# TXH-mercury/VALOR

Hardware: AMD Instinct MI355X
Metric: pretrain samples/sec (V+A+T clip) (higher is better)
Workload: dtype bf16

## Files before the change

### include/valor_hip.h

```cpp
#ifndef VALOR_HIP_H
#define VALOR_HIP_H
#include <stdint.h>
#ifdef __cplusplus
extern "C" {
#endif

#define VALOR_DT_BF16 0
#define VALOR_DT_F32 1
#define VALOR_OK 0
#define VALOR_ERR_ARG (-1)
#define VALOR_ERR_LAUNCH (-2)
#define VALOR_ACT_NONE 0
#define VALOR_ACT_GELU_ERF 1
#define VALOR_ACT_QUICK_GELU 2
#define VALOR_ACT_RELU 3
#define VALOR_ACT_TANH 4
#define VALOR_ACT_DERIV 16

int valor_gemm(void* stream, int dtype, int transA, int transB, int M, int N, int K, const void* A, int64_t lda,
               const void* B, int64_t ldb, void* C, int64_t ldc, const void* bias, int act, void* preact,
               const void* dact_aux, int64_t ldaux, float alpha, int accumulate, int out_f32, void* workspace,
               int64_t workspace_bytes, void* rowsum_out,
               int rowsum_accumulate);

typedef struct valor_gemm_policy {
    int key[12];
    int variant;
    int tr_asm;
    int fast_epilogue;
    int sched_256;
    int sched_narrow;
} valor_gemm_policy;
int valor_gemm_tuned(const valor_gemm_policy* policy, void* stream, int dtype, int transA, int transB, int M, int N, int K,
                     const void* A, int64_t lda, const void* B, int64_t ldb, void* C, int64_t ldc, const void* bias, int act,
                     void* preact, const void* dact_aux, int64_t ldaux, float alpha, int accumulate, int out_f32, void* workspace,
                     int64_t workspace_bytes, void* rowsum_out, int rowsum_accumulate);
int valor_gemm_kernel_for_tuned(const valor_gemm_policy* policy, int dtype, int transA, int transB, int M, int N, int K,
                                int heavy_epilogue);

typedef struct valor_gemm_pending { unsigned char opaque[256]; } valor_gemm_pending;
int valor_gemm_deferred(void* stream, int dtype, int transA, int transB, int M, int N, int K, const void* A, int64_t lda,
                        const void* B, int64_t ldb, void* C, int64_t ldc, const void* bias, int act, void* preact,
                        const void* dact_aux, int64_t ldaux, float alpha, int accumulate, int out_f32, void* workspace,
                        int64_t workspace_bytes, void* rowsum_out, int rowsum_accumulate, valor_gemm_pending* pending);
int valor_gemm_pending_bytes(const valor_gemm_pending* pending, int64_t* bytes);
int valor_gemm_reduce_group(void* stream, int dtype, const valor_gemm_pending* pendings, int n);

int valor_gemm_set_variant(int v);
int valor_gemm_kernel_for(int dtype, int transA, int transB, int M, int N, int K, int heavy_epilogue);
int valor_gemm_set_tr_asm(int v);
int valor_gemm_set_fast_epilogue(int v);
int valor_gemm_set_policy(int key, int value);
int valor_gemm_set_8ph_sched(int v);
int valor_gemm_set_narrow_sched(int v);
int valor_gemm_narrow_occupancy(void);
int valor_gemm_wide_occupancy(void);

typedef struct valor_xattn_seg {
    const void* q; const void* o; const void* dout; void* dq; const float* lse; const int* kv_range;
    int64_t q_bs, q_rs, o_bs, o_rs, do_bs, do_rs, dq_bs, dq_rs;
    int B, Sq;
    uint64_t seed, offset;
} valor_xattn_seg;
int valor_cross_attn_fwd_fused(void* stream, int dtype, const valor_xattn_seg* segs, int nseg, const void* k, const void* v, int H, int Skv,
                               int kv_bmod, int64_t k_bs, int64_t k_rs, int64_t v_bs, int64_t v_rs, float scale, float p_drop,
                               const uint64_t* rng_base);
int valor_cross_attn_bwd_fused(void* stream, int dtype, const valor_xattn_seg* segs, int nseg, const void* k, const void* v, void* dk, void* dv,
                               int H, int Skv, int kv_bmod, int64_t k_bs, int64_t k_rs, int64_t v_bs, int64_t v_rs, int64_t dk_bs,
                               int64_t dk_rs, int64_t dv_bs, int64_t dv_rs, float scale, float p_drop, const uint64_t* rng_base);

int valor_ln_part_blocks(void);
int valor_ln_set_variant(int v);
int valor_ln_set_nt(int v);
int valor_bdrln_fwd(void* stream, int dtype, const void* x, const void* bias, const void* residual, const void* gamma,
                    const void* beta, void* z, void* y, float* mean, float* rstd, int64_t rows, int cols, float eps,
                    float p_drop, uint64_t seed, uint64_t offset, const float* row_scale, int64_t rows_per_scale,
                    const uint64_t* rng_base);
int valor_bdrln_bwd(void* stream, int dtype, const void* dy, const void* dz_in, const void* z, const float* mean,
                    const float* rstd, const void* gamma, void* dx, void* dres, float* part_dgamma, float* part_dbeta,
                    float* part_dbias, int64_t rows, int cols, float p_drop, uint64_t seed, uint64_t offset, const float* row_scale,
                    int64_t rows_per_scale, const uint64_t* rng_base);
int valor_colsum_finalize(void* stream, int dtype, const float* part, int nparts, int cols, void* out, int out_f32,
                          int accumulate);
int valor_colsum_finalize3(void* stream, int dtype, const float* part0, void* out0, int acc0, const float* part1, void* out1,
                           int acc1, const float* part2, void* out2, int acc2, int nparts, int cols);
int valor_colsum(void* stream, int dtype, const void* x, int64_t rows, int cols, int64_t ld, float* part, void* out,
                 int out_f32, int accumulate);

int valor_attn_set_variant(int v);
int valor_attn_decode_fwd(void* stream, int dtype, const void* q, const void* k, const void* v, void* o, float* lse,
                          int B, int H, int Sq, int Skv, int64_t q_bs, int64_t q_rs, int64_t k_bs, int64_t k_rs,
                          int64_t v_bs, int64_t v_rs, int64_t o_bs, int64_t o_rs, const float* mask, int64_t mask_bs,
                          int64_t mask_rs, const int* key_row, int64_t key_row_bs, float scale);
int valor_attn_set_res_pipeline(int v);

int valor_attn_fwd(void* stream, int dtype, const void* q, const void* k, const void* v, void* o, float* lse, int B,
                   int H, int Sq, int Skv, int64_t q_bs, int64_t q_rs, int64_t k_bs, int64_t k_rs, int64_t v_bs,
                   int64_t v_rs, int64_t o_bs, int64_t o_rs, const float* mask, int64_t mask_bs, int64_t mask_rs,
                   const int* kv_range, int kv_bmod, float scale, float p_drop, uint64_t seed, uint64_t offset,
                   const uint64_t* rng_base);
int valor_attn_bwd(void* stream, int dtype, const void* q, const void* k, const void* v, const void* o, const float* lse,
                   const void* dout, void* dq, void* dk, void* dv, float* delta, int B, int H, int Sq, int Skv,
                   int64_t q_bs, int64_t q_rs, int64_t k_bs, int64_t k_rs, int64_t v_bs, int64_t v_rs, int64_t o_bs,
                   int64_t o_rs, int64_t do_bs, int64_t do_rs, int64_t dq_bs, int64_t dq_rs, int64_t dk_bs, int64_t dk_rs,
                   int64_t dv_bs, int64_t dv_rs, const float* mask, int64_t mask_bs, int64_t mask_rs, const int* kv_range,
                   int kv_bmod, float scale, float p_drop, uint64_t seed, uint64_t offset, int accumulate_dkdv,
                   const uint64_t* rng_base);

int valor_win_attn_set_variant(int v);
int valor_win_attn_workspace_floats(int B, int nW, int N, int heads);
int valor_win_attn_fwd(void* stream, int dtype, const void* qkv, void* o, float* lse, const int* rowmap, const int* rel,
                       const uint8_t* label, const void* table, int B, int nW, int N, int heads, int table_rows, int relc,
                       int rows_per_sample, float scale);
int valor_win_attn_bwd(void* stream, int dtype, const void* qkv, const void* o, const float* lse, const void* dout, void* dqkv,
                       float* delta, const int* rowmap, const int* rel, const int* rel_inv, const uint8_t* label, const void* table,
                       void* dtable, int accumulate_dtable, void* workspace, int64_t workspace_bytes, int B, int nW, int N, int heads,
                       int table_rows, int relc, int rows_per_sample, float scale);

int valor_reducer_unique_id(void* id128);
int valor_reducer_create(void** out, const void* id128, int rank, int world, int dtype, void* grad_base, const int64_t* offsets,
                         const int64_t* counts, int nbuckets, int mode);
int valor_reducer_launch_bucket(void* reducer, int bucket, void* const* compute_streams, int nstreams);
int valor_reducer_wait(void* reducer, void* stream);
int valor_reducer_destroy(void* reducer);

int valor_xent_fwd(void* stream, int dtype, const void* logits, const int64_t* labels, float* loss_rows, float* lse,
                   int64_t rows, int V, int64_t ld);
int valor_xent_bwd(void* stream, int dtype, void* logits_inout, const int64_t* labels, const float* lse,
                   const float* gscale_dev, float gmul, int64_t rows, int V, int64_t ld);
int valor_xent_smooth_fwd(void* stream, int dtype, const void* logits, const int64_t* labels, float* loss_rows, float* lse,
                          int64_t rows, int V, int64_t ld, float smoothing);
int valor_xent_smooth_bwd(void* stream, int dtype, void* logits_inout, const int64_t* labels, const float* lse,
                          const float* gscale_dev, float gmul, int64_t rows, int V, int64_t ld, float smoothing);
int valor_mean_f32(void* stream, const float* x, int64_t n, float* out);
int valor_xent_weighted_bwd(void* stream, int dtype, void* logits_inout, const int64_t* labels, const float* lse, const float* w_rows,
                            const float* gscale_dev, float gmul, int64_t rows, int V, int64_t ld);
int valor_weighted_mean_f32(void* stream, const float* x, const float* w, int64_t n, float* out);

int valor_fine_weight_softmax(void* stream, const float* raw, const float* mask, float* w, int rows, int n);
int valor_fine_weight_softmax_bwd(void* stream, const float* w, const float* dw, float* draw, int rows, int n);
int valor_fine_reduce_fwd(void* stream, const float* S, int64_t ldS, const float* maskA, const float* maskB,
                          const float* wA, const float* wB, float* score, float* A2B, float* B2A, uint8_t* idxA,
                          uint8_t* idxB, int B, int T, int Nv);
int valor_fine_scores(void* stream, const float* S, int64_t ldS, const float* maskA, const float* maskB, const float* wA,
                      const float* wB, float* score, int NA, int NB, int T, int Nv);
int valor_infonce_fwd(void* stream, const float* score, const float* k_dev, float* lse_r, float* lse_c, float* loss, int B);
int valor_infonce_bwd(void* stream, const float* score, const float* k_dev, const float* lse_r, const float* lse_c,
                      const float* g_dev, float* dscore, float* dk, float* part, int B);
int valor_fine_reduce_bwd(void* stream, int dtype, const float* dscore, const float* maskA, const float* maskB,
                          const float* wA, const float* wB, const float* A2B, const float* B2A, const uint8_t* idxA,
                          const uint8_t* idxB, void* dS, int64_t ldS, float* dwA, float* dwB, int B, int T, int Nv);
int valor_fine_fused_fwd(void* stream, const void* featA, const void* featB, const float* maskA, const float* maskB, const float* wA,
                         const float* wB, float* score, float* A2B, float* B2A, uint8_t* idxA, uint8_t* idxB, int NA, int NB, int T,
                         int Nv, int D);
int valor_fine_ds_chunk(void* stream, int dtype, const float* dscore, const float* maskA, const float* maskB, const float* wA,
                        const float* wB, const uint8_t* idxA, const uint8_t* idxB, void* dS, int64_t ldS, int a0, int na, int NB, int T,
                        int Nv);
int valor_fine_weight_grad(void* stream, const float* dscore, const float* A2B, const float* B2A, float* dwA, float* dwB, int B, int T,
                           int Nv);
int valor_fine_set_fused(int v);

int valor_retrieval_workspace_bytes(int Nt, int Nv, int64_t* bytes);
int valor_retrieval_ranks(void* stream, const float* score, int64_t ld, const int* gt_col, const int* col_ptr, const int* col_rows,
                          int nnz, float inv_temp, int dual, float* lse_row, float* lse_col, int* rank_f, int* rank_b, void* workspace,
                          int64_t workspace_bytes, int Nt, int Nv);

int valor_topk_workspace_bytes(int R, int C, int k, int64_t* bytes);
int valor_topk_rows(void* stream, const float* score, int64_t ld, int R, int C, int64_t col_base, int k, int merge, float* top_val,
                    int64_t* top_idx, void* workspace, int64_t workspace_bytes);

int valor_fp8_quantize_rows(void* stream, int dtype, const void* x, int64_t ld, int64_t rows, int cols, uint8_t* codes, float* scales);
int valor_fine_fused_fwd_fp8(void* stream, const uint8_t* codesA, const float* scaleA, const uint8_t* codesB, const float* scaleB,
                             const float* maskA, const float* maskB, const float* wA, const float* wB, float* score, int NA, int NB,
                             int T, int Nv, int D);

int valor_fine_score_pairs(void* stream, const void* featA, const float* maskA, const float* wA, const void* storeB,
                           const float* wStoreB, int64_t NS, const int64_t* cand, int64_t ld_cand, float* score, int64_t ld_score,
                           int NA, int C, int T, int Nv, int D);

int valor_adamw_chunk(void);
int valor_adamw_set_nt(int v);
int valor_adamw(void* stream, int dtype, float* master, float* exp_avg, float* exp_avg_sq, void* grad, void* param,
                const int8_t* chunk_group, int64_t n, const float* lr, const float* wd, int ngroups, float beta1,
                float beta2, float eps, int step, int correct_bias, const float* gscale_dev, int zero_grad);
int valor_adamw_counted(void* stream, int dtype, float* master, float* exp_avg, float* exp_avg_sq, void* grad, void* param,
                        const int8_t* chunk_group, const int32_t* chunk_tensor, int32_t* tensor_step, int ntensors, float* chunk_bc,
                        int64_t n, const float* lr, const float* wd, int ngroups, float beta1, float beta2, float eps,
                        int correct_bias, const float* gscale_dev, int zero_grad);
int valor_grad_norm_clip(void* stream, int dtype, const void* grad, const int8_t* chunk_group, int64_t n, float norm_mul,
                         float max_norm, float* partial, float* total_norm, float* gscale);

int valor_patchify(void* stream, int dtype, const float* in, void* out, int N, int C, int H, int W, int P, int64_t ld_out);
int valor_patchify3d(void* stream, int dtype, const float* in, void* out, int B, int F, int C, int H, int W, int P);
int valor_group_mean_fwd(void* stream, int dtype, const void* in, void* out, int64_t groups, int X, int E);
int valor_group_mean_bwd(void* stream, int dtype, const void* dout, void* din, int64_t groups, int X, int E);
int valor_assemble_tokens_fwd(void* stream, int dtype, const void* patches, const void* cls, const void* pos,
                              const void* bias, void* out, int N, int Pn, int E);
int valor_assemble_tokens_bwd(void* stream, int dtype, const void* dout, void* dpatches, void* dpos, void* dcls, int N, int Pn, int E, int accumulate);
int valor_sum_over_batch(void* stream, int dtype, const void* x, void* dsum, int N, int Tn, int E, int accumulate);
int valor_embed_fwd(void* stream, int dtype, const int64_t* ids, const void* word, const void* pos, const void* typevec,
                    void* out, int64_t n, int L, int E);
int valor_embed_bwd_word(void* stream, int dtype, const int64_t* ids, const void* dout, void* dword, int64_t n, int E, int accumulate);
int valor_add_frame_type_fwd(void* stream, int dtype, const void* in, const void* frame_emb, const void* type_emb, void* out,
                             int Bn, int F, int X, int E, int64_t out_bs, int64_t out_row_off);
int valor_add_frame_type_bwd(void* stream, int dtype, const void* dout, void* din, void* dframe, float* part, int Bn, int F,
                             int X, int E, int64_t out_bs, int64_t out_row_off);
int valor_l2norm_fwd(void* stream, int dtype, const void* x, void* y, float* norm, int64_t rows, int cols);
int valor_l2norm_bwd(void* stream, int dtype, const void* y, const void* dy, const float* norm, void* dx, int64_t rows, int cols);
int valor_gather_rows(void* stream, int dtype, const void* src, const int64_t* idx, void* out, int64_t n, int E, int64_t src_ld);
int valor_scatter_rows(void* stream, int dtype, const void* src, const int64_t* idx, void* dst, int64_t n, int E, int64_t dst_ld);
int valor_cast_from_f32(void* stream, int dtype, const float* in, void* out, int64_t n);
int valor_mask_tokens(void* stream, const int64_t* tokens, const int32_t* k, int b, int T, uint64_t seed, uint64_t offset,
                      int64_t mask_token, int64_t range_start, int64_t range_end, int64_t* tokens_out, int64_t* labels);
int valor_masked_rows(void* stream, const int64_t* labels, const int32_t* row_off, int b, int T, int G, int64_t Ttot, int64_t r0,
                      int64_t n, int64_t* idx, int64_t* lab_out);
int valor_decode_prologue(void* stream, int dtype, const int64_t* tok, const int64_t* t_dev, const void* word_emb, const void* pos_emb,
                          const void* type_row, int mask_id, int R, int J, int E, int P, int L, float neg, float* kmask, float* amask,
                          void* x, int64_t* slots_new);
int valor_beam_select(void* stream, const float* logits, int64_t ld, int64_t row_stride_s, int64_t row_stride_k, const float* lse,
                      const float* seq_logprob, const float* seq_mask, int b, int cur, int V, int beam, float* sel_val,
                      int64_t* sel_idx, float* lse_out);
int valor_sample_tokens(void* stream, const float* logits, int64_t ld, int R, int V, uint64_t seed, uint64_t offset, int64_t eos,
// ... 72 lines not shown
```

### valor_amd/csrc/attention_x.hip

```cpp
#include "attn_common.h"
#include <type_traits>
#include <stdlib.h>

DEVINL float x_exp2(float x) { return __builtin_amdgcn_exp2f(x); }

DEVINL rsrc_t x_head_rsrc(const void* base, int64_t elem_off, int rows, int64_t rs) {
    return make_rsrc((const bf16_t*)base + elem_off, (uint32_t)(((int64_t)(rows - 1) * rs + ATT_D) * 2));
}

struct XSub { int b, q0, start, len; bool valid; };
DEVINL XSub x_sub(const AttnArgs& p, int u, int kvb, int bmod, int QS, int G) {
    XSub s;
    const int j = u / QS;
    s.valid = j < G;
    s.b = kvb + (s.valid ? j : 0) * bmod;
    s.q0 = (u - j * QS) * 16;
    s.start = 0; s.len = p.Skv;
    if (p.kv_range) { s.start = p.kv_range[2 * s.b]; s.len = p.kv_range[2 * s.b + 1]; }
    return s;
}

DEVINL void x_stage_kv(rsrc_t rsK, rsrc_t rsV, char* sK, char* sV, int kv0, int krs_b, int vrs_b, int wave, int lane) {
    const int prow = lane >> 3, pch = (lane & 7) ^ prow;
#pragma unroll
// ... 47 lines not shown
    }
    const float sl2 = p.scale * LOG2E_F;
    const uint32_t thr = drop_threshold(p.p_drop);
    const float keep_scale = p.p_drop > 0.f ? 1.0f / (1.0f - p.p_drop) : 1.0f;
    int troff[4];
#pragma unroll
    for (int dt = 0; dt < 4; ++dt) troff[dt] = tr_lane_off(lane, dt);
    const int kw0 = wave * 32;
    const int NT = (p.Skv + 127) >> 7;

    constexpr bool HK_ONCE = NQS <= 4;
    uint32_t hk_[HK_ONCE ? NQS : 1];
    if (HK_ONCE) {
#pragma unroll
        for (int u = 0; u < NQS; ++u) hk_[HK_ONCE ? u : 0] = DROP ? attn_drop_headkey(p.seed, rng_off, sb_[u] * p.H + h) : 0u;
    }
    if (DB) x_stage_kv(rsK, rsV, smem + 16384, smem, 0, krs_b, vrs_b, wave, lane);
    auto tile = [&](const int t, auto stage_c) {
        constexpr int STG = decltype(stage_c)::value;
        const int kv0 = t << 7;
        char* sV = smem + STG * 32768;
        char* sK = sV + 16384;
        if (!DB) x_stage_kv(rsK, rsV, sK, sV, kv0, krs_b, vrs_b, wave, lane);
        asm volatile("s_waitcnt vmcnt(0)" ::: "memory");
        __syncthreads();
        if (DB && t + 1 < NT) {
            char* nV = smem + (STG ^ 1) * 32768;
            x_stage_kv(rsK, rsV, nV + 16384, nV, kv0 + 128, krs_b, vrs_b, wave, lane);
        }
        const int ka = kv0 + kw0;
        if (ka < p.Skv) {
            bf16x8_t kf[2][2], vfr[4];
#pragma unroll
            for (int kt = 0; kt < 2; ++kt)
#pragma unroll
                for (int dg = 0; dg < 2; ++dg) kf[kt][dg] = read_frag<bf16_t>(sK, kw0 + kt * 16 + fr, dg * 4 + g);
            if (DB) {
                TrPair tv[4];
#pragma unroll
                for (int dt = 0; dt < 4; ++dt) x_tr_issue(tv[dt], sV + kw0 * TILE_ROW_BYTES + troff[dt]);
                x_tr_wait4(tv);
#pragma unroll
                for (int dt = 0; dt < 4; ++dt) vfr[dt] = tr_frag(tv[dt]);
            } else {
#pragma unroll
                for (int dt = 0; dt < 4; ++dt) vfr[dt] = read_frag_tr_nat(sV, kw0, troff[dt]);
            }
#pragma unroll
            for (int u = 0; u < NQS; ++u) {
                const int rs0 = ss0_[u], rs1 = ss1_[u];
                if (!sv_[u] || ka + 32 <= rs0 || ka >= rs1) continue;
                f32x4_t sacc[2];
#pragma unroll
                for (int kt = 0; kt < 2; ++kt) {
                    sacc[kt] = (f32x4_t){0.f, 0.f, 0.f, 0.f};
#pragma unroll
                    for (int dg = 0; dg < 2; ++dg) sacc[kt] = Mma<bf16_t>::mma(kf[kt][dg], qf[u][dg], sacc[kt]);
                }
                float mx = -INFINITY;
                if (ka >= rs0 && ka + 32 <= rs1) {
#pragma unroll
                    for (int kt = 0; kt < 2; ++kt) {
                        sacc[kt] *= sl2;
                        mx = fmaxf(mx, fmaxf(fmaxf(sacc[kt][0], sacc[kt][1]), fmaxf(sacc[kt][2], sacc[kt][3])));
                    }
                } else {
#pragma unroll
                    for (int kt = 0; kt < 2; ++kt)
#pragma unroll
                        for (int r = 0; r < 4; ++r) {
                            const int key = ka + kt * 16 + 4 * g + r;
                            const float s = (key >= rs0 && key < rs1) ? sacc[kt][r] * sl2 : -INFINITY;
                            sacc[kt][r] = s;
                            mx = fmaxf(mx, s);
                        }
                }
                mx = fmaxf(mx, __shfl_xor(mx, 16, 64));
                mx = fmaxf(mx, __shfl_xor(mx, 32, 64));
                const float mnew = fmaxf(mrow[u], mx);
                const float alpha = x_exp2(mrow[u] - mnew);
                mrow[u] = mnew;
                float ps = 0.f;
                const int qr = sq0_[u] + fr;
                const uint32_t hk = HK_ONCE ? hk_[HK_ONCE ? u : 0] : attn_drop_headkey(p.seed, rng_off, sb_[u] * p.H + h);
                const uint32_t rowbase = (uint32_t)qr * (uint32_t)p.Skv;
#pragma unroll
                for (int kt = 0; kt < 2; ++kt) {
                    const f32x4_t sm = sacc[kt] - mnew;
#pragma unroll
                    for (int r = 0; r < 4; ++r) {
                        float pv = x_exp2(sm[r]);
                        ps += pv;
                        if (DROP) {
                            const int kloc = ka + kt * 16 + 4 * g + r - rs0;
                            pv = attn_drop_bits(hk, rowbase + (uint32_t)kloc) >= thr ? pv * keep_scale : 0.f;
                        }
                        sacc[kt][r] = pv;
                    }
                }
                lrow[u] = lrow[u] * alpha + ps;
                const bf16x8_t pf = pack_bf16x8(sacc[0], sacc[1]);
#pragma unroll
                for (int dt = 0; dt < 4; ++dt) {
                    oacc[u][dt] *= alpha;
                    oacc[u][dt] = Mma<bf16_t>::mma(vfr[dt], pf, oacc[u][dt]);
                }
            }
        }
        if (!DB) __syncthreads();
    };
    for (int t = 0; t < NT; t += DB ? 2 : 1) {
        tile(t, std::integral_constant<int, 0>{});
        if (DB && t + 1 < NT) tile(t + 1, std::integral_constant<int, 1>{});
    }
    if (DB) __syncthreads();

    float* sO = (float*)smem;
    float* sM = (float*)(smem + 16384);
    float* sL = sM + 64;
#pragma unroll
    for (int u = 0; u < NQS; ++u) {
        if (!sv_[u]) continue;
        float l = lrow[u];
        l += __shfl_xor(l, 16, 64);
        l += __shfl_xor(l, 32, 64);
        if (g == 0) { sM[wave * 16 + fr] = mrow[u]; sL[wave * 16 + fr] = l; }
#pragma unroll
        for (int dt = 0; dt < 4; ++dt)
            *(f32x4_t*)(sO + wave * 1024 + fr * 64 + (((dt * 4 + g) ^ fr) << 2)) = oacc[u][dt];
        __syncthreads();
        if (wave == (u & 3)) {
            float mw[4], M = -1e30f;
#pragma unroll
            for (int w = 0; w < 4; ++w) { mw[w] = sM[w * 16 + fr]; M = fmaxf(M, mw[w]); }
            float L = 0.f, f[4];
#pragma unroll
            for (int w = 0; w < 4; ++w) { f[w] = x_exp2(mw[w] - M); L += sL[w * 16 + fr] * f[w]; }
            const float inv = L > 0.f ? 1.0f / L : 0.f;
            const int qr = sq0_[u] + fr;
            if (qr < p.Sq) {
                bf16_t* O = (bf16_t*)p.o + (int64_t)sb_[u] * p.o_bs + (int64_t)qr * p.o_rs + h * ATT_D;
#pragma unroll
                for (int dt = 0; dt < 4; ++dt) {
                    f32x4_t a = {0.f, 0.f, 0.f, 0.f};
#pragma unroll
                    for (int w = 0; w < 4; ++w) a += *(const f32x4_t*)(sO + w * 1024 + fr * 64 + (((dt * 4 + g) ^ fr) << 2)) * f[w];
                    store4<bf16_t>(O + dt * 16 + 4 * g, a * inv);
                }
                if (g == 0 && p.lse) p.lse[((int64_t)sb_[u] * p.H + h) * p.Sq + qr] = (M + __log2f(L)) * LN2_F;
            }
        }
        __syncthreads();
    }
}

template <int NQS, bool DROP, bool ACC>
__global__ __launch_bounds__(256, 2) void attn_x_bwd_kernel(AttnArgs p) {
    const uint64_t rng_off = rng_offset(p.offset, p.rng_base);
    extern __shared__ __attribute__((aligned(16))) char smem[];
    constexpr int QIMG = NQS * 16 * TILE_ROW_BYTES;
    char* sQ = smem;
    char* sDO = smem + QIMG;
    char* sK = smem + 2 * QIMG;
    char* sV = sK + 16384;
    char* sT = sV + 16384;
    float* sLse = (float*)(sT + 4096);
    float* sDelta = sLse + NQS * 16;
    const int tid = threadIdx.x, lane = tid & 63;
    const int wave = __builtin_amdgcn_readfirstlane(tid >> 6);
    const int fr = lane & 15, g = lane >> 4;
    const int h = blockIdx.x, kvb = blockIdx.y;
    const int bmod = p.kv_bmod > 0 ? p.kv_bmod : p.B;
    const int QS = (p.Sq + 15) >> 4, G = p.B / bmod;

    const rsrc_t rsK = x_head_rsrc(p.k, (int64_t)kvb * p.k_bs + h * ATT_D, p.Skv, p.k_rs);
    const rsrc_t rsV = x_head_rsrc(p.v, (int64_t)kvb * p.v_bs + h * ATT_D, p.Skv, p.v_rs);
    const int krs_b = (int)p.k_rs * 2, vrs_b = (int)p.v_rs * 2;

    int sb_[NQS], sq0_[NQS], ss0_[NQS], ss1_[NQS];
    bool sv_[NQS];
#pragma unroll
    for (int u = 0; u < NQS; ++u) {
        const XSub t_ = x_sub(p, u, kvb, bmod, QS, G);
        sb_[u] = t_.b; sq0_[u] = t_.q0; ss0_[u] = t_.start; ss1_[u] = t_.start + t_.len; sv_[u] = t_.valid;
    }

    {
        const int prow = lane >> 3, pch = (lane & 7) ^ prow;
#pragma unroll
        for (int u = 0; u < NQS; ++u) {
            if (sv_[u]) {
                const rsrc_t rq = x_head_rsrc(p.q, (int64_t)sb_[u] * p.q_bs + h * ATT_D, p.Sq, p.q_rs);
                const rsrc_t rd = x_head_rsrc(p.dout, (int64_t)sb_[u] * p.do_bs + h * ATT_D, p.Sq, p.do_rs);
                const int piece = wave & 1;
                const int row = sq0_[u] + piece * 8 + prow;
                if (wave < 2) glds16(rq, sQ + (u * 2 + piece) * 1024, row * (int)(p.q_rs * 2) + pch * 16);
                else glds16(rd, sDO + (u * 2 + piece) * 1024, row * (int)(p.do_rs * 2) + pch * 16);
            }
        }
#pragma unroll
        for (int u = 0; u < NQS; ++u)
            if (!sv_[u]) {
                if (tid < 128) *(u32x4_t*)(sQ + u * 2048 + tid * 16) = (u32x4_t){0u, 0u, 0u, 0u};
                else *(u32x4_t*)(sDO + u * 2048 + (tid - 128) * 16) = (u32x4_t){0u, 0u, 0u, 0u};
            }
        for (int r0 = wave * 8; r0 < NQS * 16; r0 += 32) {
            const int u = r0 >> 4;
            const XSub su = x_sub(p, u, kvb, bmod, QS, G);
            const int row = su.q0 + (r0 & 15) + (lane >> 3), c = lane & 7;
            float d = 0.f;
            const bool ok = su.valid && row < p.Sq;
            if (ok) {
                const bf16_t* Ob = (const bf16_t*)p.o + (int64_t)su.b * p.o_bs + (int64_t)row * p.o_rs + h * ATT_D + c * 8;
                const bf16_t* Db = (const bf16_t*)p.dout + (int64_t)su.b * p.do_bs + (int64_t)row * p.do_rs + h * ATT_D + c * 8;
                const bf16x8_t ov = __builtin_bit_cast(bf16x8_t, *(const u32x4_t*)Ob);
                const bf16x8_t dv = __builtin_bit_cast(bf16x8_t, *(const u32x4_t*)Db);
#pragma unroll
                for (int e = 0; e < 8; ++e) d += (float)ov[e] * (float)dv[e];
            }
            d += __shfl_xor(d, 1, 64); d += __shfl_xor(d, 2, 64); d += __shfl_xor(d, 4, 64);
            if (c == 0) {
                sDelta[r0 + (lane >> 3)] = d;
                sLse[r0 + (lane >> 3)] = ok ? p.lse[((int64_t)su.b * p.H + h) * p.Sq + row] * LOG2E_F : INFINITY;
            }
        }
    }

    f32x4_t dqacc[NQS][4];
#pragma unroll
    for (int u = 0; u < NQS; ++u)
#pragma unroll
        for (int dt = 0; dt < 4; ++dt) dqacc[u][dt] = (f32x4_t){0.f, 0.f, 0.f, 0.f};

    const float sl2 = p.scale * LOG2E_F;
    const uint32_t thr = drop_threshold(p.p_drop);
    const float keep_scale = p.p_drop > 0.f ? 1.0f / (1.0f - p.p_drop) : 1.0f;
    int troff[4];
#pragma unroll
    for (int dt = 0; dt < 4; ++dt) troff[dt] = tr_lane_off(lane, dt);
    const int kw0 = wave * 32;
    char* sTw = sT + wave * 1024;
    const int tw_off = (fr * 32) + 8 * g;
    const int tr_off = (4 * g + (fr >> 2)) * 32 + 8 * (fr & 3);
    const int NT = (p.Skv + 127) >> 7;

    for (int t = 0; t < NT; ++t) {
        const int kv0 = t << 7;
        x_stage_kv(rsK, rsV, sK, sV, kv0, krs_b, vrs_b, wave, lane);
        asm volatile("s_waitcnt vmcnt(0)" ::: "memory");
        __syncthreads();
        const int ka = kv0 + kw0;
        if (ka < p.Skv) {
            bf16x8_t kf[2][2], vf[2][2];
#pragma unroll
            for (int kt = 0; kt < 2; ++kt)
#pragma unroll
                for (int dg = 0; dg < 2; ++dg) {
                    kf[kt][dg] = read_frag<bf16_t>(sK, kw0 + kt * 16 + fr, dg * 4 + g);
                    vf[kt][dg] = read_frag<bf16_t>(sV, kw0 + kt * 16 + fr, dg * 4 + g);
                }
            f32x4_t dkacc[2][4], dvacc[2][4];
#pragma unroll
            for (int kt = 0; kt < 2; ++kt)
#pragma unroll
                for (int dt = 0; dt < 4; ++dt) { dkacc[kt][dt] = (f32x4_t){0.f, 0.f, 0.f, 0.f}; dvacc[kt][dt] = dkacc[kt][dt]; }

#pragma unroll
            for (int v = 0; v < NQS / 2; ++v) {
                bool act[2];
#pragma unroll
                for (int uu = 0; uu < 2; ++uu) {
                    act[uu] = sv_[2 * v + uu] && ka + 32 > ss0_[2 * v + uu] && ka < ss1_[2 * v + uu];
                }
                if (!act[0] && !act[1]) continue;
                u32x2_t pdp[2][2], dsp[2][2];
#pragma unroll
                for (int uu = 0; uu < 2; ++uu) {
                    pdp[uu][0] = (u32x2_t){0u, 0u}; pdp[uu][1] = pdp[uu][0]; dsp[uu][0] = pdp[uu][0]; dsp[uu][1] = pdp[uu][0];
                    if (!act[uu]) continue;
                    const int u = 2 * v + uu;
                    f32x4_t sacc[2], pacc[2];
                    sacc[0] = (f32x4_t){0.f, 0.f, 0.f, 0.f}; sacc[1] = sacc[0]; pacc[0] = sacc[0]; pacc[1] = sacc[0];
#pragma unroll
                    for (int dg = 0; dg < 2; ++dg) {
                        const bf16x8_t qfr = read_frag<bf16_t>(sQ, u * 16 + fr, dg * 4 + g);
                        const bf16x8_t dfr = read_frag<bf16_t>(sDO, u * 16 + fr, dg * 4 + g);
#pragma unroll
                        for (int kt = 0; kt < 2; ++kt) {
                            sacc[kt] = Mma<bf16_t>::mma(qfr, kf[kt][dg], sacc[kt]);
                            pacc[kt] = Mma<bf16_t>::mma(dfr, vf[kt][dg], pacc[kt]);
                        }
                    }
                    const f32x4_t l4 = *(const f32x4_t*)(sLse + u * 16 + 4 * g);
                    const f32x4_t d4 = *(const f32x4_t*)(sDelta + u * 16 + 4 * g);
                    const uint32_t hk = attn_drop_headkey(p.seed, rng_off, sb_[u] * p.H + h);
                    const uint32_t row0 = (uint32_t)(sq0_[u] + 4 * g);
#pragma unroll
                    for (int kt = 0; kt < 2; ++kt) {
                        const int key = ka + kt * 16 + fr;
                        const float kout = (key >= ss0_[u] && key < ss1_[u]) ? 0.f : INFINITY;
                        f32x4_t pdv, dsv;
#pragma unroll
                        for (int r = 0; r < 4; ++r) {
                            const float prb = x_exp2(sacc[kt][r] * sl2 - l4[r] - kout);
                            float dp = pacc[kt][r];
                            float pd = prb;
                            if (DROP) {
                                const bool keep = attn_drop_bits(hk, (row0 + r) * (uint32_t)p.Skv + (uint32_t)(key - ss0_[u])) >= thr;
                                dp = keep ? dp * keep_scale : 0.f;
                                pd = keep ? prb * keep_scale : 0.f;
                            }
                            pdv[r] = pd;
                            dsv[r] = prb * (dp - d4[r]);
                        }
                        pdp[uu][kt] = (u32x2_t){pack2_bf16(pdv[0], pdv[1]), pack2_bf16(pdv[2], pdv[3])};
                        dsp[uu][kt] = (u32x2_t){pack2_bf16(dsv[0], dsv[1]), pack2_bf16(dsv[2], dsv[3])};
                    }
                    *(u32x2_t*)(sTw + tw_off) = dsp[uu][0];
                    *(u32x2_t*)(sTw + 512 + tw_off) = dsp[uu][1];
                    asm volatile("s_waitcnt lgkmcnt(0)" ::: "memory");
                    const s16x4_t t0 = lds_read_tr4(sTw + tr_off), t1 = lds_read_tr4(sTw + 512 + tr_off);
                    const bf16x8_t dst = __builtin_bit_cast(bf16x8_t, __builtin_shufflevector(t0, t1, 0, 1, 2, 3, 4, 5, 6, 7));
                    asm volatile("s_waitcnt lgkmcnt(0)" ::: "memory");
#pragma unroll
                    for (int dt = 0; dt < 4; ++dt)
                        dqacc[u][dt] = Mma<bf16_t>::mma(read_frag_tr_nat(sK, kw0, troff[dt]), dst, dqacc[u][dt]);
                }
                bf16x8_t pf[2], sf[2];
#pragma unroll
                for (int kt = 0; kt < 2; ++kt) {
                    pf[kt] = __builtin_bit_cast(bf16x8_t, (u32x4_t){pdp[0][kt][0], pdp[0][kt][1], pdp[1][kt][0], pdp[1][kt][1]});
                    sf[kt] = __builtin_bit_cast(bf16x8_t, (u32x4_t){dsp[0][kt][0], dsp[0][kt][1], dsp[1][kt][0], dsp[1][kt][1]});
                }
#pragma unroll
                for (int dt = 0; dt < 4; ++dt) {
                    const bf16x8_t dot = read_frag_tr_nat(sDO, v * 32, troff[dt]);
                    const bf16x8_t qt = read_frag_tr_nat(sQ, v * 32, troff[dt]);
#pragma unroll
                    for (int kt = 0; kt < 2; ++kt) {
                        dvacc[kt][dt] = Mma<bf16_t>::mma(dot, pf[kt], dvacc[kt][dt]);
                        dkacc[kt][dt] = Mma<bf16_t>::mma(qt, sf[kt], dkacc[kt][dt]);
                    }
                }
            }
            {
                u32x2_t oldk[2][4], oldv[2][4];
                if (ACC) {
#pragma unroll
                    for (int kt = 0; kt < 2; ++kt) {
                        const int key = ka + kt * 16 + fr;
                        const int kc = key < p.Skv ? key : p.Skv - 1;
                        const bf16_t* DK = (const bf16_t*)p.dk + (int64_t)kvb * p.dk_bs + (int64_t)kc * p.dk_rs + h * ATT_D;
                        const bf16_t* DV = (const bf16_t*)p.dv + (int64_t)kvb * p.dv_bs + (int64_t)kc * p.dv_rs + h * ATT_D;
#pragma unroll
                        for (int dt = 0; dt < 4; ++dt) {
                            oldk[kt][dt] = *(const u32x2_t*)(DK + dt * 16 + 4 * g);
                            oldv[kt][dt] = *(const u32x2_t*)(DV + dt * 16 + 4 * g);
                        }
                    }
                }
#pragma unroll
                for (int kt = 0; kt < 2; ++kt) {
                    const int key = ka + kt * 16 + fr;
                    if (key < p.Skv) {
                        bf16_t* DK = (bf16_t*)p.dk + (int64_t)kvb * p.dk_bs + (int64_t)key * p.dk_rs + h * ATT_D;
                        bf16_t* DV = (bf16_t*)p.dv + (int64_t)kvb * p.dv_bs + (int64_t)key * p.dv_rs + h * ATT_D;
#pragma unroll
                        for (int dt = 0; dt < 4; ++dt) {
                            f32x4_t ok = dkacc[kt][dt] * p.scale, ov = dvacc[kt][dt];
                            if (ACC) {
                                const u32x2_t a = oldk[kt][dt], b2 = oldv[kt][dt];
                                ok += (f32x4_t){__uint_as_float(a[0] << 16), __uint_as_float(a[0] & 0xffff0000u), __uint_as_float(a[1] << 16), __uint_as_float(a[1] & 0xffff0000u)};
                                ov += (f32x4_t){__uint_as_float(b2[0] << 16), __uint_as_float(b2[0] & 0xffff0000u), __uint_as_float(b2[1] << 16), __uint_as_float(b2[1] & 0xffff0000u)};
                            }
                            store4<bf16_t>(DK + dt * 16 + 4 * g, ok);
                            store4<bf16_t>(DV + dt * 16 + 4 * g, ov);
                        }
                    }
                }
            }
        }
        __syncthreads();
    }

    float* sR = (float*)sK;
#pragma unroll
    for (int v = 0; v < NQS / 2; ++v) {
#pragma unroll
        for (int uu = 0; uu < 2; ++uu)
#pragma unroll
            for (int dt = 0; dt < 4; ++dt)
                *(f32x4_t*)(sR + (uu * 4 + wave) * 1024 + fr * 64 + (((dt * 4 + g) ^ fr) << 2)) = dqacc[2 * v + uu][dt];
        __syncthreads();
        if (wave < 2) {
            const int qr = (wave == 0 ? sq0_[2 * v] : sq0_[2 * v + 1]) + fr;
            const bool uv = wave == 0 ? sv_[2 * v] : sv_[2 * v + 1];
            const int ubb = wave == 0 ? sb_[2 * v] : sb_[2 * v + 1];
            if (uv && qr < p.Sq) {
                bf16_t* DQ = (bf16_t*)p.dq + (int64_t)ubb * p.dq_bs + (int64_t)qr * p.dq_rs + h * ATT_D;
#pragma unroll
                for (int dt = 0; dt < 4; ++dt) {
                    f32x4_t a = {0.f, 0.f, 0.f, 0.f};
#pragma unroll
                    for (int w = 0; w < 4; ++w) a += *(const f32x4_t*)(sR + (wave * 4 + w) * 1024 + fr * 64 + (((dt * 4 + g) ^ fr) << 2));
                    store4<bf16_t>(DQ + dt * 16 + 4 * g, a * p.scale);
                }
            }
        }
        __syncthreads();
    }
}

static int x_nqs(const AttnArgs& p) {
    if (p.mask) return 0;
    const int bmod = p.kv_bmod > 0 ? p.kv_bmod : p.B;
    if (bmod <= 0 || p.B % bmod) return 0;
    const int64_t lim = (int64_t)1 << 31;
    if ((int64_t)p.Skv * p.k_rs * 2 >= lim || (int64_t)p.Skv * p.v_rs * 2 >= lim || (int64_t)p.Sq * p.q_rs * 2 >= lim) return 0;
    return (p.B / bmod) * ((p.Sq + 15) >> 4);
}

bool attn_x_fwd_launch(hipStream_t st, const AttnArgs& p) {
    const int n = x_nqs(p);
    if (n <= 0 || n > 8 || p.Skv < 128) return false;
    const int bmod = p.kv_bmod > 0 ? p.kv_bmod : p.B;
    dim3 grid(p.H, bmod);
    static const int db = [] { const char* e = getenv("VALOR_XATTN_FWD_DB"); return e ? atoi(e) : 1; }();
    const size_t lds = db ? 65536 + 1024 : 32768 + 1024;
#define X_FWD_I(N_, D_, B_)                                                                                          \
    do {                                                                                                            \
        static bool attr_set = false;                                                                               \
        if (!attr_set) {                                                                                            \
            hipFuncSetAttribute((const void*)attn_x_fwd_kernel<N_, D_, B_>, hipFuncAttributeMaxDynamicSharedMemorySize, 65536 + 1024); \
            attr_set = true;                                                                                        \
        }                                                                                                           \
        hipLaunchKernelGGL((attn_x_fwd_kernel<N_, D_, B_>), grid, dim3(256), lds, st, p);                           \
    } while (0)
#define X_FWD(N_)                                                                                                   \
    do {                                                                                                            \
        if (p.p_drop > 0.f) { if (db) X_FWD_I(N_, true, true); else X_FWD_I(N_, true, false); }                     \
        else { if (db) X_FWD_I(N_, false, true); else X_FWD_I(N_, false, false); }                                  \
    } while (0)
    if (n <= 2) X_FWD(2); else if (n <= 4) X_FWD(4); else if (n <= 6) X_FWD(6); else X_FWD(8);
#undef X_FWD
#undef X_FWD_I
    return true;
}

bool attn_x_bwd_launch(hipStream_t st, const AttnArgs& p) {
    const int n = x_nqs(p);
    if (n <= 0 || n > 4 || p.Skv < 128 || (int64_t)p.Sq * p.do_rs * 2 >= ((int64_t)1 << 31)) return false;
    const int bmod = p.kv_bmod > 0 ? p.kv_bmod : p.B;
    dim3 grid(p.H, bmod);
#define X_BWD_I(N_, D_, A_)                                                                                         \
    do {                                                                                                            \
        const size_t lds = N_ * 4096 + 32768 + 4096 + N_ * 128;                                                     \
        static bool attr_set = false;                                                                               \
        if (!attr_set) {                                                                                            \
            hipFuncSetAttribute((const void*)attn_x_bwd_kernel<N_, D_, A_>, hipFuncAttributeMaxDynamicSharedMemorySize, (int)lds); \
            attr_set = true;                                                                                        \
        }                                                                                                           \
        hipLaunchKernelGGL((attn_x_bwd_kernel<N_, D_, A_>), grid, dim3(256), lds, st, p);                           \
    } while (0)
#define X_BWD(N_)                                                                                                   \
    do {                                                                                                            \
        if (p.p_drop > 0.f) { if (p.acc_dkv) X_BWD_I(N_, true, true); else X_BWD_I(N_, true, false); }              \
        else { if (p.acc_dkv) X_BWD_I(N_, false, true); else X_BWD_I(N_, false, false); }                           \
    } while (0)
    if (n <= 2) X_BWD(2); else X_BWD(4);
#undef X_BWD
#undef X_BWD_I
    return true;
}
```

### valor_amd/csrc/attention_xu.hip

```cpp
#include "attn_common.h"

struct XuSeg {
    const void* q; const void* o; const void* dout; void* dq; const float* lse; const int* kv_range;
    int64_t q_bs, q_rs, o_bs, o_rs, do_bs, do_rs, dq_bs, dq_rs;
    int B, Sq;
    uint64_t seed, offset;
};
struct XuArgs {
    XuSeg s[2];
    const void* k; const void* v; void* dk; void* dv;
    int64_t k_bs, k_rs, v_bs, v_rs, dk_bs, dk_rs, dv_bs, dv_rs;
    int nseg, bmod, H, Skv;
    int n0, qs0, qs1, nsub;
    float scale, p_drop;
    const uint64_t* rng_base;
};

DEVINL float xu_exp2(float x) { return __builtin_amdgcn_exp2f(x); }
DEVINL rsrc_t xu_head_rsrc(const void* base, int64_t elem_off, int rows, int64_t rs) {
    return make_rsrc((const bf16_t*)base + elem_off, (uint32_t)(((int64_t)(rows - 1) * rs + ATT_D) * 2));
}

struct XuSub { int seg, b, q0, start, end; bool valid; };
DEVINL XuSub xu_sub(const XuArgs& p, int u, int kvb) {
    XuSub s;
    s.valid = u < p.nsub;
    const int uu = s.valid ? u : 0;
    s.seg = uu >= p.n0 ? 1 : 0;
    const int ul = s.seg ? uu - p.n0 : uu;
    const int qs = s.seg ? p.qs1 : p.qs0;
    const int j = ul / qs;
    s.b = kvb + j * p.bmod;
    s.q0 = (ul - j * qs) * 16;
    const int* kr = s.seg ? p.s[1].kv_range : p.s[0].kv_range;
    s.start = 0; s.end = p.Skv;
    if (kr) { s.start = kr[2 * s.b]; s.end = s.start + kr[2 * s.b + 1]; }
    return s;
}

#ifdef ATT_STAMP
#ifndef XU_STAMP_TILE
#define XU_STAMP_TILE 10
#endif
__device__ uint64_t g_xu_stamps[1024 * 4 * 16];
extern "C" int valor_attn_xu_read_stamps(void* dst, size_t bytes) {
    return (int)hipMemcpyFromSymbol(dst, HIP_SYMBOL(g_xu_stamps), bytes < sizeof(g_xu_stamps) ? bytes : sizeof(g_xu_stamps));
}
#define XU_STAMP_AT(i) do { if (t == XU_STAMP_TILE) { asm volatile("s_waitcnt lgkmcnt(0)" ::: "memory"); stamp_[i] = __builtin_amdgcn_s_memtime(); } } while (0)
#else
#define XU_STAMP_AT(i)
#endif

template <int NQS, bool DROP>
__global__ __launch_bounds__(256, 2) void attn_xu_bwd_kernel(XuArgs p) {
#ifdef ATT_STAMP
    uint64_t stamp_[12] = {0, 0, 0, 0, 0, 0, 0, 0, 0, 0, 0, 0};
    stamp_[9] = __builtin_amdgcn_s_memtime();
#endif
    const uint64_t rng_off0 = rng_offset(p.s[0].offset, p.rng_base), rng_off1 = rng_offset(p.s[1].offset, p.rng_base);
    extern __shared__ __attribute__((aligned(16))) char smem[];
    constexpr int QIMG = NQS * 16 * TILE_ROW_BYTES;
    char* sQ = smem;
    char* sDO = smem + QIMG;
    char* sK = smem + 2 * QIMG;
    char* sV = sK + 8192;
    char* sDS = sV + 8192;
    float* sLse = (float*)(sDS + NQS * 2048);
    float* sDelta = sLse + NQS * 16;
    const int tid = threadIdx.x, lane = tid & 63;
    const int wave = __builtin_amdgcn_readfirstlane(tid >> 6);
    const int fr = lane & 15, g = lane >> 4;
    const int item = blockIdx.x;
    const int h = item % p.H, kvb = item / p.H;

    const rsrc_t rsK = xu_head_rsrc(p.k, (int64_t)kvb * p.k_bs + h * ATT_D, p.Skv, p.k_rs);
    const rsrc_t rsV = xu_head_rsrc(p.v, (int64_t)kvb * p.v_bs + h * ATT_D, p.Skv, p.v_rs);
    const int krs_b = (int)p.k_rs * 2, vrs_b = (int)p.v_rs * 2;

    int sb_[NQS], sq0_[NQS], ss0_[NQS], ss1_[NQS], sg_[NQS];
    bool sv_[NQS];
#pragma unroll
    for (int u = 0; u < NQS; ++u) {
        const XuSub t_ = xu_sub(p, u, kvb);
        sb_[u] = t_.b; sq0_[u] = t_.q0; ss0_[u] = t_.start; ss1_[u] = t_.end; sv_[u] = t_.valid; sg_[u] = t_.seg;
    }

    {
        const int prow = lane >> 3, pch = (lane & 7) ^ prow;
#pragma unroll
        for (int u = 0; u < NQS; ++u) {
            if (sv_[u]) {
                const XuSeg& sg = sg_[u] ? p.s[1] : p.s[0];
                const int piece = wave & 1;
                const int row = sq0_[u] + piece * 8 + prow;
                if (wave < 2) {
                    const rsrc_t rq = xu_head_rsrc(sg.q, (int64_t)sb_[u] * sg.q_bs + h * ATT_D, sg.Sq, sg.q_rs);
                    glds16(rq, sQ + (u * 2 + piece) * 1024, row * (int)(sg.q_rs * 2) + pch * 16);
                } else {
                    const rsrc_t rd = xu_head_rsrc(sg.dout, (int64_t)sb_[u] * sg.do_bs + h * ATT_D, sg.Sq, sg.do_rs);
                    glds16(rd, sDO + (u * 2 + piece) * 1024, row * (int)(sg.do_rs * 2) + pch * 16);
                }
            } else {
                if (tid < 128) *(u32x4_t*)(sQ + u * 2048 + tid * 16) = (u32x4_t){0u, 0u, 0u, 0u};
                else *(u32x4_t*)(sDO + u * 2048 + (tid - 128) * 16) = (u32x4_t){0u, 0u, 0u, 0u};
            }
        }
        for (int r0 = wave * 8; r0 < NQS * 16; r0 += 32) {
            const int u = r0 >> 4;
            const XuSub su = xu_sub(p, u, kvb);
            const XuSeg& sg = su.seg ? p.s[1] : p.s[0];
            const int row = su.q0 + (r0 & 15) + (lane >> 3), c = lane & 7;
            float d = 0.f;
            const bool ok = su.valid && row < sg.Sq;
            if (ok) {
                const bf16_t* Ob = (const bf16_t*)sg.o + (int64_t)su.b * sg.o_bs + (int64_t)row * sg.o_rs + h * ATT_D + c * 8;
                const bf16_t* Db = (const bf16_t*)sg.dout + (int64_t)su.b * sg.do_bs + (int64_t)row * sg.do_rs + h * ATT_D + c * 8;
                const bf16x8_t ov = __builtin_bit_cast(bf16x8_t, *(const u32x4_t*)Ob);
                const bf16x8_t dv = __builtin_bit_cast(bf16x8_t, *(const u32x4_t*)Db);
#pragma unroll
                for (int e = 0; e < 8; ++e) d += (float)ov[e] * (float)dv[e];
            }
            d += __shfl_xor(d, 1, 64); d += __shfl_xor(d, 2, 64); d += __shfl_xor(d, 4, 64);
            if (c == 0) {
                sDelta[r0 + (lane >> 3)] = d;
                sLse[r0 + (lane >> 3)] = ok ? sg.lse[((int64_t)su.b * p.H + h) * sg.Sq + row] * LOG2E_F : INFINITY;
            }
        }
    }

    f32x4_t dqacc[NQS];
#pragma unroll
    for (int u = 0; u < NQS; ++u) dqacc[u] = (f32x4_t){0.f, 0.f, 0.f, 0.f};

    const float sl2 = p.scale * LOG2E_F;
    const uint32_t thr = drop_threshold(p.p_drop);
    const float keep_scale = p.p_drop > 0.f ? 1.0f / (1.0f - p.p_drop) : 1.0f;
    int troff[4];
#pragma unroll
    for (int dt = 0; dt < 4; ++dt) troff[dt] = tr_lane_off(lane, dt);
    const int troff_w = tr_lane_off(lane, wave);
    const int kw0 = wave * 16;
    const int ds_w = (kw0 + fr) * 32 + 8 * g;
    const int ds_r = (4 * g + (fr >> 2)) * 32 + 8 * (fr & 3);
    const int NT = (p.Skv + 63) >> 6;
    const int prow = lane >> 3, pch = (lane & 7) ^ prow;

#ifdef ATT_STAMP
    asm volatile("s_waitcnt vmcnt(0) lgkmcnt(0)" ::: "memory");
    stamp_[10] = __builtin_amdgcn_s_memtime();
#endif
    for (int t = 0; t < NT; ++t) {
        const int kv0 = t << 6;
        XU_STAMP_AT(0);
#pragma unroll
        for (int i = 0; i < 2; ++i) {
            const int j = wave * 2 + i;
            glds16(rsK, sK + j * 1024, (kv0 + j * 8 + prow) * krs_b + pch * 16);
            glds16(rsV, sV + j * 1024, (kv0 + j * 8 + prow) * vrs_b + pch * 16);
        }
        XU_STAMP_AT(1);
        asm volatile("s_waitcnt vmcnt(0)" ::: "memory");
        XU_STAMP_AT(2);
        __syncthreads();
        XU_STAMP_AT(3);
        const int ka = kv0 + kw0;
        bf16x8_t kf[2], vf[2];
#pragma unroll
        for (int dg = 0; dg < 2; ++dg) {
            kf[dg] = read_frag<bf16_t>(sK, kw0 + fr, dg * 4 + g);
            vf[dg] = read_frag<bf16_t>(sV, kw0 + fr, dg * 4 + g);
        }
        f32x4_t dkacc[4], dvacc[4];
#pragma unroll
        for (int dt = 0; dt < 4; ++dt) { dkacc[dt] = (f32x4_t){0.f, 0.f, 0.f, 0.f}; dvacc[dt] = dkacc[dt]; }

#pragma unroll
        for (int v = 0; v < NQS / 2; ++v) {
            bool actw[2];
            u32x2_t pdp[2], dsp[2];
#pragma unroll
            for (int uu = 0; uu < 2; ++uu) {
                const int u = 2 * v + uu;
                pdp[uu] = (u32x2_t){0u, 0u}; dsp[uu] = pdp[uu];
                const bool actt = sv_[u] && kv0 + 64 > ss0_[u] && kv0 < ss1_[u];
                actw[uu] = actt && ka + 16 > ss0_[u] && ka < ss1_[u];
                if (!actt) continue;
                if (actw[uu]) {
                    f32x4_t sacc = {0.f, 0.f, 0.f, 0.f}, pacc = {0.f, 0.f, 0.f, 0.f};
#pragma unroll
                    for (int dg = 0; dg < 2; ++dg) {
                        const bf16x8_t qfr = read_frag<bf16_t>(sQ, u * 16 + fr, dg * 4 + g);
                        const bf16x8_t dfr = read_frag<bf16_t>(sDO, u * 16 + fr, dg * 4 + g);
                        sacc = Mma<bf16_t>::mma(qfr, kf[dg], sacc);
                        pacc = Mma<bf16_t>::mma(dfr, vf[dg], pacc);
                    }
                    const f32x4_t l4 = *(const f32x4_t*)(sLse + u * 16 + 4 * g);
                    const f32x4_t d4 = *(const f32x4_t*)(sDelta + u * 16 + 4 * g);
                    const int key = ka + fr;
                    const float kout = (key >= ss0_[u] && key < ss1_[u]) ? 0.f : INFINITY;
                    uint32_t hk = 0;
                    if (DROP) {
                        const XuSeg& sg = sg_[u] ? p.s[1] : p.s[0];
                        hk = attn_drop_headkey(sg.seed, (sg_[u] ? rng_off1 : rng_off0), sb_[u] * p.H + h);
                    }
                    const uint32_t row0 = (uint32_t)(sq0_[u] + 4 * g);
                    f32x4_t pdv, dsv;
#pragma unroll
                    for (int r = 0; r < 4; ++r) {
                        const float prb = xu_exp2(sacc[r] * sl2 - l4[r] - kout);
                        float dp = pacc[r];
                        float pd = prb;
                        if (DROP) {
                            const bool keep = attn_drop_bits(hk, (row0 + r) * (uint32_t)p.Skv + (uint32_t)(key - ss0_[u])) >= thr;
                            dp = keep ? dp * keep_scale : 0.f;
                            pd = keep ? prb * keep_scale : 0.f;
                        }
                        pdv[r] = pd;
                        dsv[r] = prb * (dp - d4[r]);
                    }
                    pdp[uu] = (u32x2_t){pack2_bf16(pdv[0], pdv[1]), pack2_bf16(pdv[2], pdv[3])};
                    dsp[uu] = (u32x2_t){pack2_bf16(dsv[0], dsv[1]), pack2_bf16(dsv[2], dsv[3])};
                }
                *(u32x2_t*)(sDS + u * 2048 + ds_w) = dsp[uu];
            }
            if (actw[0] || actw[1]) {
                const bf16x8_t pf = __builtin_bit_cast(bf16x8_t, (u32x4_t){pdp[0][0], pdp[0][1], pdp[1][0], pdp[1][1]});
                const bf16x8_t sf = __builtin_bit_cast(bf16x8_t, (u32x4_t){dsp[0][0], dsp[0][1], dsp[1][0], dsp[1][1]});
#pragma unroll
                for (int dt = 0; dt < 4; ++dt) {
                    dvacc[dt] = Mma<bf16_t>::mma(read_frag_tr_nat(sDO, v * 32, troff[dt]), pf, dvacc[dt]);
                    dkacc[dt] = Mma<bf16_t>::mma(read_frag_tr_nat(sQ, v * 32, troff[dt]), sf, dkacc[dt]);
                }
            }
        }
        XU_STAMP_AT(4);
        __syncthreads();
        XU_STAMP_AT(5);
        {
            const bf16x8_t kt0 = read_frag_tr_nat(sK, 0, troff_w), kt1 = read_frag_tr_nat(sK, 32, troff_w);
#pragma unroll
            for (int u = 0; u < NQS; ++u) {
                if (!(sv_[u] && kv0 + 64 > ss0_[u] && kv0 < ss1_[u])) continue;
                const char* b = sDS + u * 2048 + ds_r;
                const s16x4_t a0 = lds_read_tr4(b), a1 = lds_read_tr4(b + 512), a2 = lds_read_tr4(b + 1024), a3 = lds_read_tr4(b + 1536);
                const bf16x8_t d0 = __builtin_bit_cast(bf16x8_t, __builtin_shufflevector(a0, a1, 0, 1, 2, 3, 4, 5, 6, 7));
                const bf16x8_t d1 = __builtin_bit_cast(bf16x8_t, __builtin_shufflevector(a2, a3, 0, 1, 2, 3, 4, 5, 6, 7));
                dqacc[u] = Mma<bf16_t>::mma(kt0, d0, dqacc[u]);
                dqacc[u] = Mma<bf16_t>::mma(kt1, d1, dqacc[u]);
            }
        }
        XU_STAMP_AT(6);
        {
            const int key = ka + fr;
            if (key < p.Skv) {
                bf16_t* DK = (bf16_t*)p.dk + (int64_t)kvb * p.dk_bs + (int64_t)key * p.dk_rs + h * ATT_D;
                bf16_t* DV = (bf16_t*)p.dv + (int64_t)kvb * p.dv_bs + (int64_t)key * p.dv_rs + h * ATT_D;
#pragma unroll
                for (int dt = 0; dt < 4; ++dt) {
                    store4<bf16_t>(DK + dt * 16 + 4 * g, dkacc[dt] * p.scale);
                    store4<bf16_t>(DV + dt * 16 + 4 * g, dvacc[dt]);
                }
            }
        }
        XU_STAMP_AT(7);
        __syncthreads();
        XU_STAMP_AT(8);
    }

#pragma unroll
    for (int u = 0; u < NQS; ++u) {
        if (!sv_[u]) continue;
        const XuSeg& sg = sg_[u] ? p.s[1] : p.s[0];
        const int qr = sq0_[u] + fr;
        if (qr < sg.Sq)
            store4<bf16_t>((bf16_t*)sg.dq + (int64_t)sb_[u] * sg.dq_bs + (int64_t)qr * sg.dq_rs + h * ATT_D + 16 * wave + 4 * g, dqacc[u] * p.scale);
    }
#ifdef ATT_STAMP
    stamp_[11] = __builtin_amdgcn_s_memtime();
    {
        const int wg = item;
        if (lane == 0 && wg < 1024) {
            uint64_t* o = g_xu_stamps + ((int64_t)wg * 4 + wave) * 16;
            for (int i = 0; i < 12; ++i) o[i] = stamp_[i];
            o[12] = __builtin_amdgcn_s_getreg((31 << 11) | 4);
            o[13] = __builtin_amdgcn_s_getreg((31 << 11) | 20);
        }
    }
#endif
}

DEVINL int xu_p_off(int fr, int b) { return fr * 128 + ((((b >> 4) ^ fr) & 7) << 4) + ((b & 8) ^ ((fr & 8))); }

template <int NQS, bool DROP>
__global__ __launch_bounds__(256, 2) void attn_xu_fwd_kernel(XuArgs p) {
    const uint64_t rng_off0 = rng_offset(p.s[0].offset, p.rng_base), rng_off1 = rng_offset(p.s[1].offset, p.rng_base);
    extern __shared__ __attribute__((aligned(16))) char smem[];
    constexpr int QIMG = NQS * 16 * TILE_ROW_BYTES;
    char* sQ = smem;
    char* sKV = smem + QIMG;
    char* sP = sKV + 32768;
    float* sMax = (float*)(sP + NQS * 2048);
    float* sSum = sMax + NQS * 64;
    const int tid = threadIdx.x, lane = tid & 63;
    const int wave = __builtin_amdgcn_readfirstlane(tid >> 6);
    const int fr = lane & 15, g = lane >> 4;
    const int h = blockIdx.x, kvb = blockIdx.y;

    const rsrc_t rsK = xu_head_rsrc(p.k, (int64_t)kvb * p.k_bs + h * ATT_D, p.Skv, p.k_rs);
    const rsrc_t rsV = xu_head_rsrc(p.v, (int64_t)kvb * p.v_bs + h * ATT_D, p.Skv, p.v_rs);
    const int krs_b = (int)p.k_rs * 2, vrs_b = (int)p.v_rs * 2;
    const int prow = lane >> 3, pch = (lane & 7) ^ prow;

    int sb_[NQS], sq0_[NQS], ss0_[NQS], ss1_[NQS], sg_[NQS];
    bool sv_[NQS];
#pragma unroll
    for (int u = 0; u < NQS; ++u) {
        const XuSub t_ = xu_sub(p, u, kvb);
        sb_[u] = t_.b; sq0_[u] = t_.q0; ss0_[u] = t_.start; ss1_[u] = t_.end; sv_[u] = t_.valid; sg_[u] = t_.seg;
    }
    for (int pc = wave; pc < 2 * NQS; pc += 4) {
        const int u = pc >> 1, piece = pc & 1;
        const XuSub su = xu_sub(p, u, kvb);
        const XuSeg& sg = su.seg ? p.s[1] : p.s[0];
        if (su.valid) {
            const rsrc_t rq = xu_head_rsrc(sg.q, (int64_t)su.b * sg.q_bs + h * ATT_D, sg.Sq, sg.q_rs);
            glds16(rq, sQ + pc * 1024, (su.q0 + piece * 8 + prow) * (int)(sg.q_rs * 2) + pch * 16);
        } else {
            *(u32x4_t*)(sQ + pc * 1024 + lane * 16) = (u32x4_t){0u, 0u, 0u, 0u};
        }
    }
    auto stage = [&](int t, char* buf) {
        const int kv0 = t << 6;
#pragma unroll
        for (int i = 0; i < 2; ++i) {
            const int j = wave * 2 + i;
            glds16(rsK, buf + j * 1024, (kv0 + j * 8 + prow) * krs_b + pch * 16);
            glds16(rsV, buf + 8192 + j * 1024, (kv0 + j * 8 + prow) * vrs_b + pch * 16);
        }
    };
    const int NT = (p.Skv + 63) >> 6;
    stage(0, sKV);

    f32x4_t oacc[NQS];
    float mrow[NQS], lrow[NQS];
#pragma unroll
    for (int u = 0; u < NQS; ++u) { oacc[u] = (f32x4_t){0.f, 0.f, 0.f, 0.f}; mrow[u] = -1e30f; lrow[u] = 0.f; }
    const float sl2 = p.scale * LOG2E_F;
    const uint32_t thr = drop_threshold(p.p_drop);
    const float keep_scale = p.p_drop > 0.f ? 1.0f / (1.0f - p.p_drop) : 1.0f;
    const int troff_w = tr_lane_off(lane, wave);
    const int kw0 = wave * 16;
    const int po[4] = {xu_p_off(fr, 8 * g), xu_p_off(fr, 8 * g + 32), xu_p_off(fr, 8 * g + 64), xu_p_off(fr, 8 * g + 96)};

    for (int t = 0; t < NT; ++t) {
        const int kv0 = t << 6;
        char* const cur = sKV + (t & 1) * 16384;
        asm volatile("s_waitcnt vmcnt(0)" ::: "memory");
        __syncthreads();
        if (t + 1 < NT) stage(t + 1, sKV + ((t + 1) & 1) * 16384);
        const int ka = kv0 + kw0;
        bf16x8_t kf[2];
#pragma unroll
        for (int dg = 0; dg < 2; ++dg) kf[dg] = read_frag<bf16_t>(cur, kw0 + fr, dg * 4 + g);
        f32x4_t sv4[NQS];
#pragma unroll
        for (int u = 0; u < NQS; ++u) {
            const bool actt = sv_[u] && kv0 + 64 > ss0_[u] && kv0 < ss1_[u];
            if (!actt) continue;
            float mx = -INFINITY;
            sv4[u] = (f32x4_t){-INFINITY, -INFINITY, -INFINITY, -INFINITY};
            if (ka + 16 > ss0_[u] && ka < ss1_[u]) {
                f32x4_t sacc = {0.f, 0.f, 0.f, 0.f};
#pragma unroll
                for (int dg = 0; dg < 2; ++dg) sacc = Mma<bf16_t>::mma(kf[dg], read_frag<bf16_t>(sQ, u * 16 + fr, dg * 4 + g), sacc);
#pragma unroll
                for (int r = 0; r < 4; ++r) {
                    const int key = ka + 4 * g + r;
                    const float s = (key >= ss0_[u] && key < ss1_[u]) ? sacc[r] * sl2 : -INFINITY;
                    sv4[u][r] = s;
                    mx = fmaxf(mx, s);
                }
                mx = fmaxf(mx, __shfl_xor(mx, 16, 64));
                mx = fmaxf(mx, __shfl_xor(mx, 32, 64));
            }
            if (g == 0) sMax[u * 64 + wave * 16 + fr] = mx;
        }
        __syncthreads();
        float alpha[NQS];
#pragma unroll
        for (int u = 0; u < NQS; ++u) {
            alpha[u] = 1.0f;
            const bool actt = sv_[u] && kv0 + 64 > ss0_[u] && kv0 < ss1_[u];
            if (!actt) continue;
            const float* mp = sMax + u * 64 + fr;
            const float mt = fmaxf(fmaxf(mp[0], mp[16]), fmaxf(mp[32], mp[48]));
            const float mnew = fmaxf(mrow[u], mt);
            alpha[u] = xu_exp2(mrow[u] - mnew);
            mrow[u] = mnew;
            float ps = 0.f;
            f32x4_t pv;
            uint32_t hk = 0;
            if (DROP) {
                const XuSeg& sg = sg_[u] ? p.s[1] : p.s[0];
                hk = attn_drop_headkey(sg.seed, (sg_[u] ? rng_off1 : rng_off0), sb_[u] * p.H + h);
            }
            const uint32_t rowbase = (uint32_t)(sq0_[u] + fr) * (uint32_t)p.Skv;
#pragma unroll
            for (int r = 0; r < 4; ++r) {
                float e = xu_exp2(sv4[u][r] - mnew);
                ps += e;
                if (DROP) e = attn_drop_bits(hk, rowbase + (uint32_t)(ka + 4 * g + r - ss0_[u])) >= thr ? e * keep_scale : 0.f;
                pv[r] = e;
            }
            ps += __shfl_xor(ps, 16, 64);
            ps += __shfl_xor(ps, 32, 64);
            lrow[u] = lrow[u] * alpha[u] + ps;
            *(u32x2_t*)(sP + u * 2048 + xu_p_off(fr, (kw0 + 4 * g) * 2)) = (u32x2_t){pack2_bf16(pv[0], pv[1]), pack2_bf16(pv[2], pv[3])};
        }
        __syncthreads();
        {
            const bf16x8_t vt0 = read_frag_tr_nat(cur + 8192, 0, troff_w), vt1 = read_frag_tr_nat(cur + 8192, 32, troff_w);
#pragma unroll
            for (int u = 0; u < NQS; ++u) {
                if (!(sv_[u] && kv0 + 64 > ss0_[u] && kv0 < ss1_[u])) continue;
                const char* b = sP + u * 2048;
                const u32x2_t a0 = *(const u32x2_t*)(b + po[0]), a1 = *(const u32x2_t*)(b + po[1]), a2 = *(const u32x2_t*)(b + po[2]),
                              a3 = *(const u32x2_t*)(b + po[3]);
                const bf16x8_t p0 = __builtin_bit_cast(bf16x8_t, (u32x4_t){a0[0], a0[1], a1[0], a1[1]});
                const bf16x8_t p1 = __builtin_bit_cast(bf16x8_t, (u32x4_t){a2[0], a2[1], a3[0], a3[1]});
                oacc[u] *= alpha[u];
                oacc[u] = Mma<bf16_t>::mma(vt0, p0, oacc[u]);
                oacc[u] = Mma<bf16_t>::mma(vt1, p1, oacc[u]);
            }
        }
    }
    __syncthreads();
#pragma unroll
    for (int u = 0; u < NQS; ++u)
        if (g == 0) sSum[u * 64 + wave * 16 + fr] = lrow[u];
    __syncthreads();
#pragma unroll
    for (int u = 0; u < NQS; ++u) {
        if (!sv_[u]) continue;
        const XuSeg& sg = sg_[u] ? p.s[1] : p.s[0];
        const float* lp = sSum + u * 64 + fr;
        const float L = (lp[0] + lp[16]) + (lp[32] + lp[48]);
        const float inv = L > 0.f ? 1.0f / L : 0.f;
        const int qr = sq0_[u] + fr;
        if (qr < sg.Sq) {
            store4<bf16_t>((bf16_t*)sg.o + (int64_t)sb_[u] * sg.o_bs + (int64_t)qr * sg.o_rs + h * ATT_D + 16 * wave + 4 * g, oacc[u] * inv);
            if (wave == 0 && g == 0) ((float*)sg.lse)[((int64_t)sb_[u] * p.H + h) * sg.Sq + qr] = (mrow[u] + __log2f(L)) * LN2_F;
        }
    }
}

static int g_xu_on = [] { const char* e = getenv("VALOR_ATTN_XFUSED"); return e ? atoi(e) : 1; }();

struct valor_xattn_seg_c {
    const void* q; const void* o; const void* dout; void* dq; const float* lse; const int* kv_range;
    int64_t q_bs, q_rs, o_bs, o_rs, do_bs, do_rs, dq_bs, dq_rs;
    int B, Sq;
    uint64_t seed, offset;
};

static int xu_fill(XuArgs& p, int dtype, const void* segs_, int nseg, const void* k, const void* v, int H, int Skv, int kv_bmod, int64_t k_bs,
                   int64_t k_rs, int64_t v_bs, int64_t v_rs, float scale, float p_drop, bool bwd) {
    const valor_xattn_seg_c* segs = (const valor_xattn_seg_c*)segs_;
    if (dtype != VALOR_DT_BF16 || !g_xu_on) return VALOR_ERR_ARG;
    if (!segs || nseg < 1 || nseg > 2 || !k || !v || H <= 0 || Skv < 64 || kv_bmod <= 0) return VALOR_ERR_ARG;
    if ((k_rs & 7) || (v_rs & 7) || (k_bs & 7) || (v_bs & 7) || ((uintptr_t)k & 15) || ((uintptr_t)v & 15)) return VALOR_ERR_ARG;
    const int64_t lim = (int64_t)1 << 31;
    if ((int64_t)Skv * k_rs * 2 >= lim || (int64_t)Skv * v_rs * 2 >= lim) return VALOR_ERR_ARG;
    p.nseg = nseg; p.bmod = kv_bmod; p.H = H; p.Skv = Skv; p.scale = scale; p.p_drop = p_drop;
    p.k = k; p.v = v;
    p.k_bs = k_bs; p.k_rs = k_rs; p.v_bs = v_bs; p.v_rs = v_rs;
    int nsub = 0;
    for (int i = 0; i < nseg; ++i) {
        const valor_xattn_seg_c& s = segs[i];
        if (!s.q || !s.o || !s.lse || s.B <= 0 || s.Sq <= 0 || s.B % kv_bmod) return VALOR_ERR_ARG;
        if ((s.q_rs & 7) || (s.q_bs & 7) || ((uintptr_t)s.q & 15) || (int64_t)s.Sq * s.q_rs * 2 >= lim) return VALOR_ERR_ARG;
        if (bwd) {
            if (!s.dout || !s.dq) return VALOR_ERR_ARG;
            if ((s.o_rs & 7) || (s.o_bs & 7) || (s.do_rs & 7) || (s.do_bs & 7) || (s.dq_rs & 3) || (s.dq_bs & 3)) return VALOR_ERR_ARG;
            if (((uintptr_t)s.o & 15) || ((uintptr_t)s.dout & 15) || (int64_t)s.Sq * s.do_rs * 2 >= lim) return VALOR_ERR_ARG;
        } else if ((s.o_rs & 3) || (s.o_bs & 3)) return VALOR_ERR_ARG;
        XuSeg& d = p.s[i];
        d.q = s.q; d.o = s.o; d.dout = s.dout; d.dq = s.dq; d.lse = s.lse; d.kv_range = s.kv_range;
        d.q_bs = s.q_bs; d.q_rs = s.q_rs; d.o_bs = s.o_bs; d.o_rs = s.o_rs; d.do_bs = s.do_bs; d.do_rs = s.do_rs; d.dq_bs = s.dq_bs; d.dq_rs = s.dq_rs;
        d.B = s.B; d.Sq = s.Sq; d.seed = s.seed; d.offset = s.offset;
        const int qs = (s.Sq + 15) >> 4, n = (s.B / kv_bmod) * qs;
        if (i == 0) { p.qs0 = qs; p.n0 = n; } else p.qs1 = qs;
        nsub += n;
    }
    if (nseg == 1) p.qs1 = 1;
    p.nsub = nsub;
    if (nsub > 10) return VALOR_ERR_ARG;
    return VALOR_OK;
}

extern "C" int valor_cross_attn_fwd_fused(void* stream, int dtype, const void* segs, int nseg, const void* k, const void* v, int H, int Skv,
                                          int kv_bmod, int64_t k_bs, int64_t k_rs, int64_t v_bs, int64_t v_rs, float scale, float p_drop,
                                          const uint64_t* rng_base) {
    XuArgs p = {};
    const int rc = xu_fill(p, dtype, segs, nseg, k, v, H, Skv, kv_bmod, k_bs, k_rs, v_bs, v_rs, scale, p_drop, false);
    if (rc != VALOR_OK) return rc;
    p.rng_base = rng_base;
    hipStream_t st = (hipStream_t)stream;
    dim3 grid(H, kv_bmod);
    const int nsub = p.nsub;
#define XUF_I(N_, D_)                                                                                               \
    do {                                                                                                            \
        const size_t lds = 2 * N_ * 2048 + 32768 + 2 * N_ * 256;                                                    \
        static bool attr_set = false;                                                                               \
        if (!attr_set) {                                                                                            \
            hipFuncSetAttribute((const void*)attn_xu_fwd_kernel<N_, D_>, hipFuncAttributeMaxDynamicSharedMemorySize, (int)lds); \
            attr_set = true;                                                                                        \
        }                                                                                                           \
        hipLaunchKernelGGL((attn_xu_fwd_kernel<N_, D_>), grid, dim3(256), lds, st, p);                              \
    } while (0)
#define XUF(N_) do { if (p_drop > 0.f) XUF_I(N_, true); else XUF_I(N_, false); } while (0)
    if (nsub <= 4) XUF(4); else if (nsub <= 6) XUF(6); else if (nsub <= 8) XUF(8); else XUF(10);
#undef XUF
#undef XUF_I
    return valor_launch_status();
}

extern "C" int valor_cross_attn_bwd_fused(void* stream, int dtype, const void* segs, int nseg, const void* k, const void* v, void* dk, void* dv,
                                          int H, int Skv, int kv_bmod, int64_t k_bs, int64_t k_rs, int64_t v_bs, int64_t v_rs, int64_t dk_bs,
                                          int64_t dk_rs, int64_t dv_bs, int64_t dv_rs, float scale, float p_drop, const uint64_t* rng_base) {
    if (!dk || !dv || (dk_rs & 3) || (dv_rs & 3) || (dk_bs & 3) || (dv_bs & 3)) return VALOR_ERR_ARG;
    XuArgs p = {};
    const int rc = xu_fill(p, dtype, segs, nseg, k, v, H, Skv, kv_bmod, k_bs, k_rs, v_bs, v_rs, scale, p_drop, true);
    if (rc != VALOR_OK) return rc;
    p.dk = dk; p.dv = dv; p.rng_base = rng_base;
    p.dk_bs = dk_bs; p.dk_rs = dk_rs; p.dv_bs = dv_bs; p.dv_rs = dv_rs;
    const int nsub = p.nsub;
    hipStream_t st = (hipStream_t)stream;
    const int n_items = H * kv_bmod;
#define XU_I(N_, D_)                                                                                                \
    do {                                                                                                            \
        const size_t lds = 3 * N_ * 2048 + 16384 + N_ * 128;                                                        \
        static bool attr_set = false;                                                                               \
        if (!attr_set) {                                                                                            \
            hipFuncSetAttribute((const void*)attn_xu_bwd_kernel<N_, D_>, hipFuncAttributeMaxDynamicSharedMemorySize, (int)lds); \
            attr_set = true;                                                                                        \
        }                                                                                                           \
        hipLaunchKernelGGL((attn_xu_bwd_kernel<N_, D_>), dim3(n_items), dim3(256), lds, st, p);                     \
    } while (0)
#define XU(N_) do { if (p_drop > 0.f) XU_I(N_, true); else XU_I(N_, false); } while (0)
    if (nsub <= 4) XU(4); else if (nsub <= 6) XU(6); else if (nsub <= 8) XU(8); else XU(10);
#undef XU
#undef XU_I
    return valor_launch_status();
}
```

### valor_amd/csrc/attn_common.h

```cpp
#pragma once
#include "mma.h"

#define ATT_D 64
#define LOG2E_F 1.44269504088896340736f
#define LN2_F 0.69314718055994530942f

struct AttnArgs {
    const void* q; const void* k; const void* v; void* o; float* lse;
    const void* dout; void* dq; void* dk; void* dv; float* delta;
    const float* mask; const int* kv_range;
    int B, H, Sq, Skv;
    int64_t q_bs, q_rs, k_bs, k_rs, v_bs, v_rs, o_bs, o_rs;
    int64_t do_bs, do_rs, dq_bs, dq_rs, dk_bs, dk_rs, dv_bs, dv_rs;
    int64_t mask_bs, mask_rs;
    int kv_bmod;
    int acc_dkv;
    float scale, p_drop;
    uint64_t seed, offset;
    const uint64_t* rng_base;
    const int* key_row;
    int64_t key_row_bs;
};

template <typename T> DEVINL float fexp(float x);
template <> DEVINL float fexp<float>(float x) { return expf(x); }
template <> DEVINL float fexp<bf16_t>(float x) { return __expf(x); }

DEVINL bf16x8_t pack_bf16x8(f32x4_t a, f32x4_t b) {
    u32x4_t r;
    r[0] = pack2_bf16(a[0], a[1]);
    r[1] = pack2_bf16(a[2], a[3]);
    r[2] = pack2_bf16(b[0], b[1]);
    r[3] = pack2_bf16(b[2], b[3]);
    return __builtin_bit_cast(bf16x8_t, r);
}


DEVINL uint32_t mix32(uint32_t x) {
    x ^= x >> 16; x *= 0x7feb352du; x ^= x >> 15; x *= 0x846ca68bu; x ^= x >> 16;
    return x;
}
DEVINL uint32_t attn_drop_headkey(uint64_t seed, uint64_t offset, int head) {
    uint32_t k = mix32((uint32_t)offset + (uint32_t)head * 0x9E3779B9u);
    k = mix32(k ^ (uint32_t)(offset >> 32) ^ (uint32_t)seed);
    return mix32(k + (uint32_t)(seed >> 32));
}
DEVINL uint32_t attn_drop_bits(uint32_t hk, uint32_t local) {
    uint32_t x = local ^ hk;
    x = __umul24(x, 0x9E3779u) + (hk >> 7);
    x ^= x >> 15;
    x = __umul24(x, 0x85EBCBu) + hk;
    x ^= x >> 13;
    return x;
}

template <bool DROP, bool WANT_P>
DEVINL void softmax_bwd4(const f32x4_t sa, const f32x4_t pa, const f32x4_t m4, const f32x4_t l4, const f32x4_t d4, float sl2, uint32_t hk,
                         uint32_t e0, uint32_t estride, uint32_t thr, float keep_scale, f32x4_t& pd, f32x4_t& ds) {
    const f32x4_t sc = sa * sl2 + (m4 - l4);
    f32x4_t prb;
#pragma unroll
    for (int r = 0; r < 4; ++r) prb[r] = __builtin_amdgcn_exp2f(sc[r]);
    f32x4_t dp = pa;
    pd = prb;
    if (DROP) {
#pragma unroll
        for (int r = 0; r < 4; ++r) {
            const bool keep = attn_drop_bits(hk, e0 + (uint32_t)r * estride) >= thr;
            dp[r] = keep ? dp[r] * keep_scale : 0.f;
            if (WANT_P) pd[r] = keep ? prb[r] * keep_scale : 0.f;
        }
    }
    ds = prb * (dp - d4);
}
DEVINL f32x4_t splat4(float x) { return (f32x4_t){x, x, x, x}; }

bool attn_res_fwd_launch(hipStream_t st, const AttnArgs& p);
bool attn_res_bwd_launch(hipStream_t st, const AttnArgs& p);
bool attn_x_fwd_launch(hipStream_t st, const AttnArgs& p);
bool attn_x_bwd_launch(hipStream_t st, const AttnArgs& p);
```

### valor_amd/kernels.py

```python
import os

import torch

from . import lib
from .lib import ACT_NONE, DT_BF16, DT_F32

_WS = {}
_WS_BYTES = 256 << 20
RNG_BASE = 0


def dt_of(t):
    if t.dtype == torch.bfloat16:
        return DT_BF16
    if t.dtype == torch.float32:
        return DT_F32
    raise TypeError(f"valor_amd kernels support bf16 / fp32 only, got {t.dtype}")


def _stream():
    return torch.cuda.current_stream().cuda_stream


def _ptr(t):
# ... 202 lines not shown
    ref = dy if dy is not None else dz_in
    _check_gpu(dy, dz_in, z, gamma)
    cols = ref.shape[-1]
    rows = ref.numel() // cols
    nb = part_blocks()
    ws = workspace(ref.device)
    need = 3 * nb * cols
    assert ws.numel() >= need
    pg = ws[0:nb * cols] if (want_dgamma and dy is not None) else None
    pb = ws[nb * cols:2 * nb * cols] if (want_dbeta and dy is not None) else None
    px = ws[2 * nb * cols:3 * nb * cols] if want_dbias else None
    dres = torch.empty_like(ref)
    dx = torch.empty_like(ref) if (p_drop > 0.0 or separate_dx or row_scale is not None) else dres
    lib.call("valor_bdrln_bwd", _stream(), dt_of(ref), _ptr(dy), _ptr(dz_in), _ptr(z), _ptr(mean), _ptr(rstd),
             _ptr(gamma), _ptr(dx), _ptr(dres), _ptr(pg), _ptr(pb), _ptr(px), rows, cols, float(p_drop), int(seed),
             int(offset), _ptr(row_scale), int(rows_per_scale), RNG_BASE)
    outs, args = [], []
    for part, sink in zip((pg, pb, px), sinks):
        if part is None:
            outs.append(None); args += [0, 0, 0]
        elif sink is not None:
            outs.append(None); args += [_ptr(part), _ptr(sink), 1]
        else:
            o = torch.empty(cols, dtype=ref.dtype, device=ref.device)
            outs.append(o); args += [_ptr(part), _ptr(o), 0]
    if any(a for a in args[0::3]):
        lib.call("valor_colsum_finalize3", _stream(), dt_of(ref), *args, nb, cols)
    return dx, dres, outs[0], outs[1], outs[2]


def colsum(x, out=None, accumulate=False):
    _check_gpu(x, out)
    rows, cols = x.shape
    ld = _rowmajor(x)
    if out is None:
        out = torch.empty(cols, dtype=x.dtype, device=x.device)
        accumulate = False
    ws = workspace(x.device)
    assert ws.numel() >= part_blocks() * cols
    lib.call("valor_colsum", _stream(), dt_of(x), _ptr(x), rows, cols, ld, _ptr(ws), _ptr(out), 0, int(accumulate))
    return out


def _bsr(t):
    assert t.dim() == 3 and t.stride(2) == 1
    return t.stride(0), t.stride(1)


def attn_fwd(q, k, v, n_heads, *, mask=None, kv_range=None, kv_bmod=0, scale=None, p_drop=0.0, seed=0, offset=0, o=None, lse=None):
    _check_gpu(q, k, v, mask, kv_range)
    B, Sq, E = q.shape
    Skv = k.shape[1]
    assert E == n_heads * 64, "head_dim is fixed at 64"
    if scale is None:
        scale = 0.125
    if o is None:
        o = torch.empty((B, Sq, E), dtype=q.dtype, device=q.device)
    if lse is None:
        lse = torch.empty((B, n_heads, Sq), dtype=torch.float32, device=q.device)
    assert o.shape == (B, Sq, E) and lse.shape == (B, n_heads, Sq) and lse.is_contiguous()
    qb, qr = _bsr(q); kb, kr = _bsr(k); vb, vr = _bsr(v); ob, orr = _bsr(o)
    mb = mr = 0
    if mask is not None:
        assert mask.dtype == torch.float32 and mask.dim() == 3 and mask.stride(2) == 1
        mb, mr = (mask.stride(0) if mask.shape[0] > 1 else 0), mask.stride(1)
    if kv_range is not None:
        assert kv_range.dtype == torch.int32 and kv_range.shape == (B, 2) and kv_range.is_contiguous()
    lib.call("valor_attn_fwd", _stream(), dt_of(q), _ptr(q), _ptr(k), _ptr(v), _ptr(o), _ptr(lse), B, n_heads, Sq, Skv,
             qb, qr, kb, kr, vb, vr, ob, orr, _ptr(mask), mb, mr, _ptr(kv_range), int(kv_bmod), float(scale),
             float(p_drop), int(seed), int(offset), RNG_BASE)
    return o, lse


def attn_decode(q, k, v, n_heads, *, mask=None, key_row=None, scale=0.125, o=None):
    _check_gpu(q, k, v, mask, key_row)
    B, Sq, E = q.shape
    Skv = k.shape[1]
    assert E == n_heads * 64, "head_dim is fixed at 64"
    if o is None:
        o = torch.empty((B, Sq, E), dtype=q.dtype, device=q.device)
    qb, qr = _bsr(q); kb, kr = _bsr(k); vb, vr = _bsr(v); ob, orr = _bsr(o)
    mb = mr = 0
    if mask is not None:
        assert mask.dtype == torch.float32 and mask.dim() == 3 and mask.stride(2) == 1
        mb, mr = (mask.stride(0) if mask.shape[0] > 1 else 0), mask.stride(1)
    rb = 0
    if key_row is not None:
        assert key_row.dtype == torch.int32 and key_row.shape == (B, Skv) and key_row.stride(1) == 1
        rb = key_row.stride(0)
    lib.call("valor_attn_decode_fwd", _stream(), dt_of(q), _ptr(q), _ptr(k), _ptr(v), _ptr(o), None, B, n_heads, Sq, Skv,
             qb, qr, kb, kr, vb, vr, ob, orr, _ptr(mask), mb, mr, _ptr(key_row), rb, float(scale))
    return o


def attn_bwd(q, k, v, o, lse, dout, n_heads, *, dq=None, dk=None, dv=None, mask=None, kv_range=None, kv_bmod=0,
             scale=None, p_drop=0.0, seed=0, offset=0, accumulate_kv=False):
    _check_gpu(q, k, v, o, dout, mask, kv_range)
    B, Sq, E = q.shape
    Skv = k.shape[1]
    if scale is None:
        scale = 0.125
    if dq is None:
        dq = torch.empty((B, Sq, E), dtype=q.dtype, device=q.device)
    if dk is None:
        dk = torch.empty((k.shape[0], Skv, E), dtype=q.dtype, device=q.device)
    if dv is None:
        dv = torch.empty((v.shape[0], Skv, E), dtype=q.dtype, device=q.device)
    delta = torch.empty((B, n_heads, Sq), dtype=torch.float32, device=q.device)
    qb, qr = _bsr(q); kb, kr = _bsr(k); vb, vr = _bsr(v); ob, orr = _bsr(o); gb, gr = _bsr(dout)
    dqb, dqr = _bsr(dq); dkb, dkr = _bsr(dk); dvb, dvr = _bsr(dv)
    mb = mr = 0
    if mask is not None:
        mb, mr = (mask.stride(0) if mask.shape[0] > 1 else 0), mask.stride(1)
    lib.call("valor_attn_bwd", _stream(), dt_of(q), _ptr(q), _ptr(k), _ptr(v), _ptr(o), _ptr(lse), _ptr(dout), _ptr(dq),
             _ptr(dk), _ptr(dv), _ptr(delta), B, n_heads, Sq, Skv, qb, qr, kb, kr, vb, vr, ob, orr, gb, gr,
             dqb, dqr, dkb, dkr, dvb, dvr, _ptr(mask), mb, mr, _ptr(kv_range), int(kv_bmod), float(scale),
             float(p_drop), int(seed), int(offset), int(accumulate_kv), RNG_BASE)
    return dq, dk, dv


def _xattn_segs(segs, kv_bmod, bwd):
    arr = (lib.XattnSeg * len(segs))()
    for i, sg in enumerate(segs):
        q, o = sg["q"], sg["o"]
        _check_gpu(q, o, sg["lse"], sg.get("kv_range"))
        a = arr[i]
        a.q, a.o, a.lse, a.kv_range = _ptr(q), _ptr(o), _ptr(sg["lse"]), _ptr(sg.get("kv_range"))
        (a.q_bs, a.q_rs), (a.o_bs, a.o_rs) = _bsr(q), _bsr(o)
        if bwd:
            do, dq = sg["dout"], sg["dq"]
            _check_gpu(do, dq)
            a.dout, a.dq = _ptr(do), _ptr(dq)
            (a.do_bs, a.do_rs), (a.dq_bs, a.dq_rs) = _bsr(do), _bsr(dq)
        a.B, a.Sq, a.seed, a.offset = q.shape[0], q.shape[1], int(sg.get("seed", 0)), int(sg.get("offset", 0))
    return arr


def _xattn_domain(segs, k, kv_bmod):
    if k.dtype != torch.bfloat16 or not (1 <= len(segs) <= 2) or k.shape[1] < 64 or kv_bmod <= 0:
        return False
    nsub = sum((sg["q"].shape[0] // kv_bmod) * ((sg["q"].shape[1] + 15) // 16) for sg in segs)
    return not (nsub > 10 or any(sg["q"].shape[0] % kv_bmod for sg in segs) or os.environ.get("VALOR_ATTN_XFUSED", "1") == "0")


def _xattn_call(name, *args):
    rc = getattr(lib.load(), name)(*args)
    if rc == -1:
        return False
    if rc != 0:
        raise lib.ValorHipError(f"{name} failed with code {rc}")
    return True


def cross_attn_fwd_fused(segs, k, v, n_heads, kv_bmod, *, scale=0.125, p_drop=0.0):
    if not _xattn_domain(segs, k, kv_bmod):
        return False
    import ctypes
    arr = _xattn_segs(segs, kv_bmod, False)
    kb, kr = _bsr(k); vb, vr = _bsr(v)
    return _xattn_call("valor_cross_attn_fwd_fused", _stream(), DT_BF16, ctypes.cast(arr, ctypes.c_void_p), len(segs), _ptr(k), _ptr(v),
                       n_heads, k.shape[1], int(kv_bmod), kb, kr, vb, vr, float(scale), float(p_drop), RNG_BASE)


def cross_attn_bwd_fused(segs, k, v, dk, dv, n_heads, kv_bmod, *, scale=0.125, p_drop=0.0):
    if not _xattn_domain(segs, k, kv_bmod):
        return False
    arr = _xattn_segs(segs, kv_bmod, True)
    kb, kr = _bsr(k); vb, vr = _bsr(v); dkb, dkr = _bsr(dk); dvb, dvr = _bsr(dv)
    import ctypes
    return _xattn_call("valor_cross_attn_bwd_fused", _stream(), DT_BF16, ctypes.cast(arr, ctypes.c_void_p), len(segs), _ptr(k), _ptr(v), _ptr(dk),
                       _ptr(dv), n_heads, k.shape[1], int(kv_bmod), kb, kr, vb, vr, dkb, dkr, dvb, dvr, float(scale), float(p_drop), RNG_BASE)


def win_attn_fwd(qkv, geo, table, n_heads, B):
    _check_gpu(qkv, table, geo["rowmap"], geo["rel"], geo["label"])
    C = n_heads * 32
    assert qkv.is_contiguous() and qkv.shape == (B * geo["rows"], 3 * C) and table.is_contiguous() and table.shape[1] == n_heads
    o = torch.empty((qkv.shape[0], C), dtype=qkv.dtype, device=qkv.device)
    lse = torch.empty((B * geo["nW"], n_heads, geo["N"]), dtype=torch.float32, device=qkv.device)
    lib.call("valor_win_attn_fwd", _stream(), dt_of(qkv), _ptr(qkv), _ptr(o), _ptr(lse), _ptr(geo["rowmap"]), _ptr(geo["rel"]),
             _ptr(geo["label"]), _ptr(table), B, geo["nW"], geo["N"], n_heads, table.shape[0], geo["relc"], geo["rows"], 32 ** -0.5)
    return o, lse


def win_attn_bwd(qkv, o, lse, dout, geo, table, n_heads, B, dtable=None):
    _check_gpu(qkv, o, dout, table, dtable)
    assert dout.is_contiguous() and dout.shape == o.shape
    dqkv = torch.empty_like(qkv)
    delta = torch.empty_like(lse)
    acc = dtable is not None
    if dtable is None:
        dtable = torch.empty_like(table)
    need = lib.load().valor_win_attn_workspace_floats(B, geo["nW"], geo["N"], n_heads)
    if need < 0:
        raise lib.ValorHipError("window attention workspace too large")
    ws = workspace(qkv.device, max(_WS_BYTES, need * 4))
    lib.call("valor_win_attn_bwd", _stream(), dt_of(qkv), _ptr(qkv), _ptr(o), _ptr(lse), _ptr(dout), _ptr(dqkv), _ptr(delta),
             _ptr(geo["rowmap"]), _ptr(geo["rel"]), _ptr(geo["rel_inv"]), _ptr(geo["label"]), _ptr(table), _ptr(dtable), int(acc), _ptr(ws),
             ws.numel() * 4,
             B, geo["nW"], geo["N"], n_heads, table.shape[0], geo["relc"], geo["rows"], 32 ** -0.5)
    return dqkv, (None if acc else dtable)


def patchify3d(video_f32, P, out_dtype):
    _check_gpu(video_f32)
    assert video_f32.dtype == torch.float32 and video_f32.is_contiguous()
    B, F, C, H, W = video_f32.shape
    out = torch.empty((B * F * (H // P) * (W // P), C * 2 * P * P), dtype=out_dtype, device=video_f32.device)
    lib.call("valor_patchify3d", _stream(), dt_of(out), _ptr(video_f32), _ptr(out), B, F, C, H, W, P)
    return out


def group_mean_fwd(x2d, X):
    _check_gpu(x2d)
    assert x2d.is_contiguous() and x2d.shape[0] % X == 0
    out = torch.empty((x2d.shape[0] // X, x2d.shape[1]), dtype=x2d.dtype, device=x2d.device)
    lib.call("valor_group_mean_fwd", _stream(), dt_of(x2d), _ptr(x2d), _ptr(out), out.shape[0], X, x2d.shape[1])
    return out


def group_mean_bwd(dout, X):
    _check_gpu(dout)
    dout = dout.contiguous()
    din = torch.empty((dout.shape[0] * X, dout.shape[1]), dtype=dout.dtype, device=dout.device)
    lib.call("valor_group_mean_bwd", _stream(), dt_of(dout), _ptr(dout), _ptr(din), dout.shape[0], X, dout.shape[1])
    return din


def mask_tokens(tokens, k, seed, offset, mask_token, range_start, range_end):
    _check_gpu(tokens, k)
    assert tokens.dtype == torch.int64 and tokens.is_contiguous() and tokens.dim() == 2
    assert k.dtype == torch.int32 and k.is_contiguous() and k.numel() == tokens.shape[0]
    b, T = tokens.shape
    out, labels = torch.empty_like(tokens), torch.empty_like(tokens)
    lib.call("valor_mask_tokens", _stream(), _ptr(tokens), _ptr(k), b, T, int(seed), int(offset), int(mask_token), int(range_start),
             int(range_end), _ptr(out), _ptr(labels))
    return out, labels


def masked_rows(labels, row_off, n, G=1, Ttot=None, r0=0, idx=None, lab_out=None):
    _check_gpu(labels, row_off, idx, lab_out)
    assert labels.dtype == torch.int64 and labels.is_contiguous() and labels.dim() == 2
    assert row_off.dtype == torch.int32 and row_off.is_contiguous() and row_off.numel() == labels.shape[0]
    b, T = labels.shape
    if idx is None:
        idx = torch.empty(G * n, dtype=torch.int64, device=labels.device)
    if lab_out is None:
        lab_out = torch.empty(G * n, dtype=torch.int64, device=labels.device)
    for t in (idx, lab_out):
        assert t.dtype == torch.int64 and t.is_contiguous() and t.numel() == G * n
    lib.call("valor_masked_rows", _stream(), _ptr(labels), _ptr(row_off), b, T, G, T if Ttot is None else int(Ttot), int(r0), int(n),
             _ptr(idx), _ptr(lab_out))
    return idx, lab_out


def _caption_rows(seq, clip_idx):
    assert seq.dtype == torch.int64 and seq.dim() == 2 and (seq.stride(1) == 1 or seq.shape[1] == 1)
    R, L = seq.shape
    assert clip_idx.dtype == torch.int32 and clip_idx.is_contiguous() and clip_idx.numel() == R
    return R, L, seq.stride(0) if R > 1 else L


def caption_reward(seq, eos, vocab, clip_idx, tables, reward, cider=None, bleu=None):
    import ctypes
    _check_gpu(seq, clip_idx, reward, cider, bleu)
    R, L, ld = _caption_rows(seq, clip_idx)
    for t in (reward, cider, bleu):
        assert t is None or (t.dtype == torch.float64 and t.is_contiguous() and t.numel() == R)
    lib.call("valor_caption_reward", _stream(), _ptr(seq), ld, R, L, int(eos), int(vocab), _ptr(clip_idx), ctypes.addressof(tables),
             _ptr(reward), _ptr(cider), _ptr(bleu))


def caption_metrics(seq, eos, vocab, clip_idx, tables, cider, rouge, bleu, counts, summary):
    import ctypes
    _check_gpu(seq, clip_idx, cider, rouge, bleu, counts, summary)
    R, L, ld = _caption_rows(seq, clip_idx)
    for t, n in ((cider, R), (rouge, R), (bleu, 4 * R)):
        assert t.dtype == torch.float64 and t.is_contiguous() and t.numel() == n
    assert counts.dtype == torch.int32 and counts.is_contiguous() and counts.numel() == 10 * R
    assert summary.dtype == torch.int64 and summary.is_contiguous() and summary.numel() == 16
    lib.call("valor_caption_metrics", _stream(), _ptr(seq), ld, R, L, int(eos), int(vocab), _ptr(clip_idx), ctypes.addressof(tables),
             _ptr(cider), _ptr(rouge), _ptr(bleu), _ptr(counts), _ptr(summary))


def sample_tokens(logits, seed, offset, eos, unfinished, tok, sents, logprobs):
    _check_gpu(logits, unfinished, tok, sents, logprobs)
    assert logits.dtype == torch.float32 and logits.dim() == 2 and logits.stride(1) == 1
    assert unfinished.dtype == torch.bool and unfinished.is_contiguous() and tok.dtype == torch.int64 and tok.is_contiguous()
    assert sents.dtype == torch.int64 and logprobs.dtype == torch.float32 and sents.dim() == logprobs.dim() == 1
    R, V = logits.shape
    assert unfinished.numel() == tok.numel() == sents.numel() == logprobs.numel() == R
    lib.call("valor_sample_tokens", _stream(), _ptr(logits), logits.stride(0), R, V, int(seed), int(offset), int(eos), _ptr(unfinished), _ptr(tok),
             _ptr(sents), sents.stride(0), _ptr(logprobs), logprobs.stride(0))


def sample_tokens_filtered(logits, seed, offset, eos, unfinished, tok, sents, logprobs, inv_temperature=1.0, top_k=0, top_p=1.0, kept=None,
                           cut=None):
    _check_gpu(logits, unfinished, tok, sents, logprobs, kept, cut)
    assert logits.dtype == torch.float32 and logits.dim() == 2 and logits.stride(1) == 1
    assert unfinished.dtype == torch.bool and unfinished.is_contiguous() and tok.dtype == torch.int64 and tok.is_contiguous()
    assert sents.dtype == torch.int64 and logprobs.dtype == torch.float32 and sents.dim() == logprobs.dim() == 1
    R, V = logits.shape
    assert unfinished.numel() == tok.numel() == sents.numel() == logprobs.numel() == R
    assert kept is None or (kept.dtype == torch.int32 and kept.is_contiguous() and kept.numel() == R)
    assert cut is None or (cut.dtype == torch.float32 and cut.is_contiguous() and cut.numel() == R)
    lib.call("valor_sample_tokens_filtered", _stream(), _ptr(logits), logits.stride(0), R, V, int(seed), int(offset), int(eos),
             float(inv_temperature), int(top_k), float(top_p), _ptr(unfinished), _ptr(tok), _ptr(sents), sents.stride(0), _ptr(logprobs),
             logprobs.stride(0), None if kept is None else _ptr(kept), None if cut is None else _ptr(cut))


def _constrain_rows(logits, hist, t, active, b, hist_stride_s, hist_stride_k):
    assert logits.dtype == torch.float32 and logits.dim() == 2 and logits.stride(1) == 1
    R, V = logits.shape
    t = int(t)
    if hist is not None:
        assert hist.dtype == torch.int64 and hist.stride(-1) == 1 and hist.shape[-1] >= t
        if hist_stride_s is None:
            assert hist.dim() == 2 and hist.shape[0] >= R
            hist_stride_s = hist.stride(0)
    else:
        assert t == 0
    b = R if b is None else int(b)
    if hist is not None and t > 0 and R > 0:
        last = ((min(R, b) - 1) * int(hist_stride_s) + ((R - 1) // b) * int(hist_stride_k) + t - 1) if b >= 1 else 0
# ... 117 lines not shown
```

### valor_amd/lib.py

```python
import ctypes
import os

_HERE = os.path.dirname(os.path.abspath(__file__))
LIB_PATH = os.environ.get("VALOR_HIP_LIB") or os.path.join(_HERE, "libvalor_hip.so")

DT_BF16 = 0
DT_F32 = 1

ACT_NONE, ACT_GELU_ERF, ACT_QUICK_GELU, ACT_RELU, ACT_TANH = 0, 1, 2, 3, 4
ACT_DERIV = 16

_c = ctypes
_vp, _i, _i64, _u64, _f = _c.c_void_p, _c.c_int, _c.c_int64, _c.c_uint64, _c.c_float

class GemmPolicy(_c.Structure):
    _fields_ = [("key", _i * 12), ("variant", _i), ("tr_asm", _i), ("fast_epilogue", _i), ("sched_256", _i), ("sched_narrow", _i)]
    KEYS = dict(nt_min_k=0, splitk_bf16=1, min_tiles=2, nt_min_tiles=3, raster=4, store=5, nta=6, nn_min_k=7, narrow=8, mfma32=9, wide=10, skinny=11)

    @classmethod
    def make(cls, **kw):
        p = cls()
        for i in range(12):
            p.key[i] = -1
        p.variant = p.tr_asm = p.fast_epilogue = p.sched_256 = p.sched_narrow = -1
        for k, v in kw.items():
            if k in cls.KEYS:
                p.key[cls.KEYS[k]] = int(v)
            else:
                setattr(p, k, int(v))
        return p


class XattnSeg(_c.Structure):
    _fields_ = [("q", _vp), ("o", _vp), ("dout", _vp), ("dq", _vp), ("lse", _vp), ("kv_range", _vp),
                ("q_bs", _i64), ("q_rs", _i64), ("o_bs", _i64), ("o_rs", _i64), ("do_bs", _i64), ("do_rs", _i64), ("dq_bs", _i64), ("dq_rs", _i64),
                ("B", _i), ("Sq", _i), ("seed", _u64), ("offset", _u64)]


class RewardTables(_c.Structure):
    POINTERS = ("g_keys", "g_idf", "clip_ref_ptr", "ref_key_ptr", "ref_keys", "ref_vals", "ref_norm", "ref_bigrams", "ref_tokens",
                "clip_bleu_ptr", "bleu_keys", "bleu_cnt")
    _fields_ = [(k, _vp) for k in POINTERS] + [("ref_len", _c.c_double), ("n_global", _c.c_int32), ("n_clips", _c.c_int32)]


class CapevalTables(_c.Structure):
    POINTERS = RewardTables.POINTERS + ("ref_sym_ptr", "ref_syms")
    _fields_ = [(k, _vp) for k in POINTERS] + [("ref_len", _c.c_double), ("n_global", _c.c_int32), ("n_clips", _c.c_int32)]


class CapevalSummary(_c.Structure):
    _fields_ = [("value", _c.c_double * 6), ("total", _c.c_int64 * 10)]


SIGNATURES = {
    "valor_gemm": [_vp, _i, _i, _i, _i, _i, _i, _vp, _i64, _vp, _i64, _vp, _i64, _vp, _i, _vp, _vp, _i64,
                   _f, _i, _i, _vp, _i64, _vp, _i],
    "valor_gemm_tuned": [_vp, _vp, _i, _i, _i, _i, _i, _i, _vp, _i64, _vp, _i64, _vp, _i64, _vp, _i, _vp, _vp, _i64,
                         _f, _i, _i, _vp, _i64, _vp, _i],
    "valor_gemm_kernel_for_tuned": [_vp, _i, _i, _i, _i, _i, _i, _i],
    "valor_gemm_deferred": [_vp, _i, _i, _i, _i, _i, _i, _vp, _i64, _vp, _i64, _vp, _i64, _vp, _i, _vp, _vp, _i64,
                            _f, _i, _i, _vp, _i64, _vp, _i, _vp],
    "valor_gemm_pending_bytes": [_vp, _vp],
    "valor_gemm_reduce_group": [_vp, _i, _vp, _i],
    "valor_gemm_set_variant": [_i],
    "valor_gemm_kernel_for": [_i, _i, _i, _i, _i, _i, _i],
    "valor_gemm_set_tr_asm": [_i],
    "valor_gemm_set_fast_epilogue": [_i],
    "valor_gemm_set_policy": [_i, _i],
    "valor_gemm_set_8ph_sched": [_i],
    "valor_gemm_set_narrow_sched": [_i],
    "valor_gemm_narrow_occupancy": [],
    "valor_gemm_wide_occupancy": [],
    "valor_ln_part_blocks": [],
    "valor_ln_set_variant": [_i],
    "valor_ln_set_nt": [_i],
    "valor_bdrln_fwd": [_vp, _i, _vp, _vp, _vp, _vp, _vp, _vp, _vp, _vp, _vp, _i64, _i, _f, _f, _u64, _u64, _vp, _i64, _vp],
    "valor_bdrln_bwd": [_vp, _i, _vp, _vp, _vp, _vp, _vp, _vp, _vp, _vp, _vp, _vp, _vp, _i64, _i, _f, _u64, _u64, _vp, _i64, _vp],
    "valor_patchify3d": [_vp, _i, _vp, _vp, _i, _i, _i, _i, _i, _i],
    "valor_group_mean_fwd": [_vp, _i, _vp, _vp, _i64, _i, _i],
    "valor_group_mean_bwd": [_vp, _i, _vp, _vp, _i64, _i, _i],
    "valor_win_attn_workspace_floats": [_i, _i, _i, _i],
    "valor_win_attn_set_variant": [_i],
    "valor_win_attn_fwd": [_vp, _i, _vp, _vp, _vp, _vp, _vp, _vp, _vp, _i, _i, _i, _i, _i, _i, _i, _f],
    "valor_win_attn_bwd": [_vp, _i, _vp, _vp, _vp, _vp, _vp, _vp, _vp, _vp, _vp, _vp, _vp, _vp, _i, _vp, _i64, _i, _i, _i, _i, _i, _i, _i, _f],
    "valor_colsum_finalize": [_vp, _i, _vp, _i, _i, _vp, _i, _i],
    "valor_colsum_finalize3": [_vp, _i, _vp, _vp, _i, _vp, _vp, _i, _vp, _vp, _i, _i, _i],
    "valor_attn_set_variant": [_i],
    "valor_attn_set_res_pipeline": [_i],
    "valor_attn_fwd": [_vp, _i, _vp, _vp, _vp, _vp, _vp, _i, _i, _i, _i, _i64, _i64, _i64, _i64, _i64, _i64, _i64, _i64,
                       _vp, _i64, _i64, _vp, _i, _f, _f, _u64, _u64, _vp],
    "valor_attn_decode_fwd": [_vp, _i, _vp, _vp, _vp, _vp, _vp, _i, _i, _i, _i, _i64, _i64, _i64, _i64, _i64, _i64, _i64, _i64,
                              _vp, _i64, _i64, _vp, _i64, _f],
    "valor_attn_bwd": [_vp, _i, _vp, _vp, _vp, _vp, _vp, _vp, _vp, _vp, _vp, _vp, _i, _i, _i, _i,
                       _i64, _i64, _i64, _i64, _i64, _i64, _i64, _i64, _i64, _i64, _i64, _i64, _i64, _i64, _i64, _i64,
                       _vp, _i64, _i64, _vp, _i, _f, _f, _u64, _u64, _i, _vp],
    "valor_cross_attn_fwd_fused": [_vp, _i, _vp, _i, _vp, _vp, _i, _i, _i, _i64, _i64, _i64, _i64, _f, _f, _vp],
    "valor_cross_attn_bwd_fused": [_vp, _i, _vp, _i, _vp, _vp, _vp, _vp, _i, _i, _i, _i64, _i64, _i64, _i64, _i64, _i64, _i64, _i64, _f, _f, _vp],
    "valor_reducer_unique_id": [_vp],
    "valor_reducer_create": [_vp, _vp, _i, _i, _i, _vp, _vp, _vp, _i, _i],
    "valor_reducer_launch_bucket": [_vp, _i, _vp, _i],
    "valor_reducer_wait": [_vp, _vp],
    "valor_reducer_destroy": [_vp],
    "valor_xent_fwd": [_vp, _i, _vp, _vp, _vp, _vp, _i64, _i, _i64],
    "valor_xent_bwd": [_vp, _i, _vp, _vp, _vp, _vp, _f, _i64, _i, _i64],
    "valor_xent_smooth_fwd": [_vp, _i, _vp, _vp, _vp, _vp, _i64, _i, _i64, _f],
    "valor_xent_smooth_bwd": [_vp, _i, _vp, _vp, _vp, _vp, _f, _i64, _i, _i64, _f],
    "valor_fine_weight_softmax": [_vp, _vp, _vp, _vp, _i, _i],
    "valor_fine_weight_softmax_bwd": [_vp, _vp, _vp, _vp, _i, _i],
    "valor_fine_reduce_fwd": [_vp, _vp, _i64, _vp, _vp, _vp, _vp, _vp, _vp, _vp, _vp, _vp, _i, _i, _i],
    "valor_fine_scores": [_vp, _vp, _i64, _vp, _vp, _vp, _vp, _vp, _i, _i, _i, _i],
    "valor_infonce_fwd": [_vp, _vp, _vp, _vp, _vp, _vp, _i],
    "valor_infonce_bwd": [_vp, _vp, _vp, _vp, _vp, _vp, _vp, _vp, _vp, _i],
    "valor_fine_reduce_bwd": [_vp, _i, _vp, _vp, _vp, _vp, _vp, _vp, _vp, _vp, _vp, _vp, _i64, _vp, _vp, _i, _i, _i],
    "valor_fine_fused_fwd": [_vp, _vp, _vp, _vp, _vp, _vp, _vp, _vp, _vp, _vp, _vp, _vp, _i, _i, _i, _i, _i],
    "valor_fine_ds_chunk": [_vp, _i, _vp, _vp, _vp, _vp, _vp, _vp, _vp, _vp, _i64, _i, _i, _i, _i, _i],
    "valor_fine_weight_grad": [_vp, _vp, _vp, _vp, _vp, _vp, _i, _i, _i],
    "valor_fine_set_fused": [_i],
    "valor_retrieval_workspace_bytes": [_i, _i, _c.POINTER(_i64)],
    "valor_retrieval_ranks": [_vp, _vp, _i64, _vp, _vp, _vp, _i, _f, _i, _vp, _vp, _vp, _vp, _vp, _i64, _i, _i],
    "valor_topk_workspace_bytes": [_i, _i, _i, _c.POINTER(_i64)],
    "valor_topk_rows": [_vp, _vp, _i64, _i, _i, _i64, _i, _i, _vp, _vp, _vp, _i64],
    "valor_fp8_quantize_rows": [_vp, _i, _vp, _i64, _i64, _i, _vp, _vp],
    "valor_fine_fused_fwd_fp8": [_vp, _vp, _vp, _vp, _vp, _vp, _vp, _vp, _vp, _vp, _i, _i, _i, _i, _i],
    "valor_fine_score_pairs": [_vp, _vp, _vp, _vp, _vp, _vp, _i64, _vp, _i64, _vp, _i64, _i, _i, _i, _i, _i],
    "valor_adamw_chunk": [],
    "valor_adamw_set_nt": [_i],
    "valor_adamw": [_vp, _i, _vp, _vp, _vp, _vp, _vp, _vp, _i64, _c.POINTER(_f), _c.POINTER(_f), _i, _f, _f, _f, _i, _i, _vp, _i],
    "valor_adamw_counted": [_vp, _i, _vp, _vp, _vp, _vp, _vp, _vp, _vp, _vp, _i, _vp, _i64, _c.POINTER(_f), _c.POINTER(_f), _i, _f, _f, _f,
                            _i, _vp, _i],
    "valor_grad_norm_clip": [_vp, _i, _vp, _vp, _i64, _f, _f, _vp, _vp, _vp],
    "valor_patchify": [_vp, _i, _vp, _vp, _i, _i, _i, _i, _i, _i64],
    "valor_assemble_tokens_fwd": [_vp, _i, _vp, _vp, _vp, _vp, _vp, _i, _i, _i],
    "valor_assemble_tokens_bwd": [_vp, _i, _vp, _vp, _vp, _vp, _i, _i, _i, _i],
    "valor_sum_over_batch": [_vp, _i, _vp, _vp, _i, _i, _i, _i],
    "valor_embed_fwd": [_vp, _i, _vp, _vp, _vp, _vp, _vp, _i64, _i, _i],
    "valor_embed_bwd_word": [_vp, _i, _vp, _vp, _vp, _i64, _i, _i],
    "valor_add_frame_type_fwd": [_vp, _i, _vp, _vp, _vp, _vp, _i, _i, _i, _i, _i64, _i64],
    "valor_add_frame_type_bwd": [_vp, _i, _vp, _vp, _vp, _vp, _i, _i, _i, _i, _i64, _i64],
    "valor_l2norm_fwd": [_vp, _i, _vp, _vp, _vp, _i64, _i],
    "valor_l2norm_bwd": [_vp, _i, _vp, _vp, _vp, _vp, _i64, _i],
    "valor_gather_rows": [_vp, _i, _vp, _vp, _vp, _i64, _i, _i64],
    "valor_decode_prologue": [_vp, _i, _vp, _vp, _vp, _vp, _vp, _i, _i, _i, _i, _i, _i, _f, _vp, _vp, _vp, _vp],
    "valor_beam_select": [_vp, _vp, _i64, _i64, _i64, _vp, _vp, _vp, _i, _i, _i, _i, _vp, _vp, _vp],
    "valor_scatter_rows": [_vp, _i, _vp, _vp, _vp, _i64, _i, _i64],
    "valor_cast_from_f32": [_vp, _i, _vp, _vp, _i64],
    "valor_mask_tokens": [_vp, _vp, _vp, _i, _i, _u64, _u64, _i64, _i64, _i64, _vp, _vp],
    "valor_masked_rows": [_vp, _vp, _vp, _i, _i, _i, _i64, _i64, _i64, _vp, _vp],
    "valor_dact_mul": [_vp, _i, _vp, _vp, _vp, _i64, _i],
    "valor_mean_f32": [_vp, _vp, _i64, _vp],
    "valor_xent_weighted_bwd": [_vp, _i, _vp, _vp, _vp, _vp, _vp, _f, _i64, _i, _i64],
    "valor_weighted_mean_f32": [_vp, _vp, _vp, _i64, _vp],
    "valor_sample_tokens": [_vp, _vp, _i64, _i, _i, _u64, _u64, _i64, _vp, _vp, _vp, _i64, _vp, _i64],
    "valor_sample_tokens_filtered": [_vp, _vp, _i64, _i, _i, _u64, _u64, _i64, _f, _i, _f, _vp, _vp, _vp, _i64, _vp, _i64, _vp, _vp],
    "valor_logits_constrain": [_vp, _vp, _i64, _i, _i, _vp, _i64, _i64, _i, _i, _i64, _f, _f, _i, _i, _vp, _i, _vp],
    "valor_trie_constrain": [_vp, _vp, _i64, _i, _i, _vp, _i64, _i64, _i, _i, _i64, _vp, _vp, _vp, _vp, _vp, _i, _i, _i, _vp],
    "valor_caption_reward": [_vp, _vp, _i64, _i, _i, _i64, _i, _vp, _vp, _vp, _vp, _vp],
    "valor_caption_metrics": [_vp, _vp, _i64, _i, _i, _i64, _i, _vp, _vp, _vp, _vp, _vp, _vp, _vp],
    "valor_rowdot_fwd": [_vp, _i, _vp, _vp, _vp, _vp, _i64, _i],
    "valor_rowdot_bwd": [_vp, _i, _vp, _vp, _vp, _vp, _vp, _vp, _i64, _i],
    "valor_colsum": [_vp, _i, _vp, _i64, _i, _i64, _vp, _vp, _i, _i],
    "valor_fbank": [_vp, _vp, _i, _i64, _vp, _vp, _i, _i, _i, _i, _i, _i, _i, _vp, _vp, _vp, _vp, _vp, _i, _f, _f, _vp],
    "valor_frames_prepare": [_vp, _vp, _i64, _vp, _vp, _i, _i, _i, _c.POINTER(_f), _c.POINTER(_f), _vp],
    "valor_meter_update": [_vp, _vp, _i, _c.POINTER(_vp), _c.POINTER(_c.c_int32), _i, _f, _f],
    "valor_arena_grad_stats": [_vp, _i, _vp, _vp, _vp, _vp, _i, _i64, _i, _f, _vp, _vp, _vp],
    "valor_arena_update_stats": [_vp, _vp, _vp, _vp, _vp, _vp, _vp, _vp, _i, _i64, _c.POINTER(_f), _i, _f, _vp, _vp, _vp, _vp],
    "valor_ema_update": [_vp, _vp, _vp, _i64, _f, _i, _vp, _vp],
    "valor_ema_set_nt": [_i],
}
STATS_FIELDS = ("g_sumsq", "g_absmax", "g_nonfinite", "g_norm", "w_sumsq", "u_sumsq", "w_norm", "u_ratio")
METER_FIELDS = ("last", "ema", "sum", "count", "min", "max", "nonfinite", "reserved")
METER_MAX_SRC = 32
TRIE_FLOOR = _c.c_float(-1e30).value

_lib = None


class ValorHipError(RuntimeError):
    pass


def load():
    global _lib
    if _lib is not None:
        return _lib
    if not os.path.exists(LIB_PATH):
        raise ValorHipError(
            f"{LIB_PATH} not found: run `python -m valor_amd.build` (hipcc --offload-arch=gfx950). "
            "valor_amd has no CPU / eager fallback by design.")
    import torch
    lib = ctypes.CDLL(LIB_PATH)
    for name, argtypes in SIGNATURES.items():
        fn = getattr(lib, name)
        fn.argtypes = argtypes
        fn.restype = _i
    _lib = lib
    return lib


def call(name, *args):
    rc = getattr(load(), name)(*args)
    if rc != 0:
        raise ValorHipError(f"{name} failed with code {rc}")
    return rc
```

### valor_amd/ops.py

```python
import math
import os
import weakref

import torch
from torch.autograd import Function

from . import kernels as K
from . import lib
from .lib import ACT_NONE

_st = K._stream
_p = K._ptr
_dt = K.dt_of


class DropoutState:
    seed = 1234
    offset = 0
    base = None
    begun = False
    STEP_STRIDE = 1 << 40

    @classmethod
    def reset(cls, seed, offset=0):
# ... 390 lines not shown
        dx, dres, _, _, dbias = K.bdrln_bwd(None, dz.contiguous(), None, None, None, None, p_drop=p_drop, seed=seed,
                                            offset=off, want_dgamma=False, want_dbeta=False, want_dbias=has_b,
                                            sinks=(None, None, sb), row_scale=ctx.rs[0], rows_per_scale=ctx.rs[1])
        if sb is not None:
            _sunk(ctx.params[0])
        return dx, dbias, (dres if has_r else None), None, None, None


def bias_dropout_residual(x, bias, residual, p_drop, row_scale=None, rows_per_scale=0):
    return BiasDropResFn.apply(x, bias, residual, p_drop, row_scale, rows_per_scale)


class SelfAttnFn(Function):

    @staticmethod
    def forward(ctx, qkv, n_heads, mask, p_drop):
        B, S, E3 = qkv.shape
        E = E3 // 3
        seed = off = 0
        if p_drop > 0:
            seed, off = DropoutState.draw_elems(B * n_heads * S * S)
        q, k, v = qkv[:, :, :E], qkv[:, :, E:2 * E], qkv[:, :, 2 * E:]
        o, lse = K.attn_fwd(q, k, v, n_heads, mask=mask, scale=1.0 / math.sqrt(64), p_drop=p_drop, seed=seed, offset=off)
        ctx.save_for_backward(qkv, o, lse, mask)
        ctx.cfg = (n_heads, p_drop, seed, off)
        return o

    @staticmethod
    def backward(ctx, do):
        qkv, o, lse, mask = ctx.saved_tensors
        n_heads, p_drop, seed, off = ctx.cfg
        E = qkv.shape[2] // 3
        dqkv = torch.empty_like(qkv)
        q, k, v = qkv[:, :, :E], qkv[:, :, E:2 * E], qkv[:, :, 2 * E:]
        K.attn_bwd(q, k, v, o, lse, do.contiguous(), n_heads, dq=dqkv[:, :, :E], dk=dqkv[:, :, E:2 * E], dv=dqkv[:, :, 2 * E:],
                   mask=mask, scale=1.0 / math.sqrt(64), p_drop=p_drop, seed=seed, offset=off)
        return dqkv, None, None, None


def self_attention(qkv, n_heads, mask=None, p_drop=0.0):
    return SelfAttnFn.apply(qkv, n_heads, mask, p_drop)


class StaticGen:
    REGISTRY = weakref.WeakValueDictionary()

    def __init__(self):
        self.gen = 0
        self.ptrs = []

    def register(self, tensors):
        self.release()
        self.ptrs = [t.data_ptr() for t in tensors]
        for q in self.ptrs:
            StaticGen.REGISTRY[q] = self

    def release(self):
        for q in self.ptrs:
            StaticGen.REGISTRY.pop(q, None)
        self.ptrs = []

    @staticmethod
    def seen(t):
        g = StaticGen.REGISTRY.get(t.data_ptr())
        return None if g is None else (g, g.gen)

    @staticmethod
    def check(tag):
        if tag is not None and tag[0].gen != tag[1]:
            raise RuntimeError("valor_amd: the static cross-attention K|V buffers were rewritten by a later training forward before this backward "
                               "ran (one forward per backward with VALOR_KV_STREAM=1; set VALOR_KV_STREAM=0 to keep several graphs alive)")


class CrossAttnFn(Function):

    @staticmethod
    def forward(ctx, q, kv, n_heads, kv_range, kv_bmod, p_drop, slot=None):
        ctx.slot = slot
        B, T, E = q.shape
        seed = off = 0
        if p_drop > 0:
            seed, off = DropoutState.draw_elems(B * n_heads * T * kv.shape[1])
        k, v = kv[:, :, :E], kv[:, :, E:]
        q = q.contiguous()
        o, lse = K.attn_fwd(q, k, v, n_heads, kv_range=kv_range, kv_bmod=kv_bmod, scale=1.0 / math.sqrt(64),
                            p_drop=p_drop, seed=seed, offset=off)
        ctx.save_for_backward(q, kv, o, lse, kv_range)
        ctx.cfg = (n_heads, kv_bmod, p_drop, seed, off)
        ctx.static_gen = StaticGen.seen(kv)
        return o

    @staticmethod
    def backward(ctx, do):
        StaticGen.check(ctx.static_gen)
        q, kv, o, lse, kv_range = ctx.saved_tensors
        n_heads, kv_bmod, p_drop, seed, off = ctx.cfg
        E = q.shape[2]
        slot = ctx.slot
        acc = slot is not None and slot.buf is not None
        dkv = slot.buf if acc else torch.empty_like(kv)
        dq, _, _ = K.attn_bwd(q, kv[:, :, :E], kv[:, :, E:], o, lse, do.contiguous(), n_heads, dk=dkv[:, :, :E],
                              dv=dkv[:, :, E:], kv_range=kv_range, kv_bmod=kv_bmod, scale=1.0 / math.sqrt(64),
                              p_drop=p_drop, seed=seed, offset=off, accumulate_kv=acc)
        if slot is not None and not acc:
            slot.buf = dkv
        return dq, (None if acc else dkv), None, None, None, None, None


def cross_attention(q, kv, n_heads, kv_range=None, kv_bmod=0, p_drop=0.0, grad_slot=None):
    return CrossAttnFn.apply(q, kv, n_heads, kv_range, kv_bmod, p_drop, grad_slot)


class SegSelfAttnFn(Function):

    @staticmethod
    def forward(ctx, qkv2d, n_heads, segs, p_drop):
        R, E3 = qkv2d.shape
        E = E3 // 3
        o = torch.empty((R, E), dtype=qkv2d.dtype, device=qkv2d.device)
        lses, rng = [], []
        for (r0, B, T, mask) in segs:
            seed = off = 0
            if p_drop > 0:
                seed, off = DropoutState.draw_elems(B * n_heads * T * T)
            v3 = qkv2d[r0:r0 + B * T].view(B, T, E3)
            lse = torch.empty((B, n_heads, T), dtype=torch.float32, device=qkv2d.device)
            K.attn_fwd(v3[:, :, :E], v3[:, :, E:2 * E], v3[:, :, 2 * E:], n_heads, mask=mask, scale=1.0 / math.sqrt(64), p_drop=p_drop,
                       seed=seed, offset=off, o=o[r0:r0 + B * T].view(B, T, E), lse=lse)
            lses.append(lse); rng.append((seed, off))
        ctx.save_for_backward(qkv2d, o, *lses)
        ctx.cfg = (n_heads, segs, p_drop, rng)
        return o

    @staticmethod
    def backward(ctx, do):
        qkv2d, o, *lses = ctx.saved_tensors
        n_heads, segs, p_drop, rng = ctx.cfg
        E = qkv2d.shape[1] // 3
        do = do.contiguous()
        dqkv = torch.empty_like(qkv2d)
        for (r0, B, T, mask), lse, (seed, off) in zip(segs, lses, rng):
            v3 = qkv2d[r0:r0 + B * T].view(B, T, 3 * E)
            d3 = dqkv[r0:r0 + B * T].view(B, T, 3 * E)
            K.attn_bwd(v3[:, :, :E], v3[:, :, E:2 * E], v3[:, :, 2 * E:], o[r0:r0 + B * T].view(B, T, E), lse,
                       do[r0:r0 + B * T].view(B, T, E), n_heads, dq=d3[:, :, :E], dk=d3[:, :, E:2 * E], dv=d3[:, :, 2 * E:],
                       mask=mask, scale=1.0 / math.sqrt(64), p_drop=p_drop, seed=seed, offset=off)
        return dqkv, None, None, None


def seg_self_attention(qkv2d, n_heads, segs, p_drop=0.0):
    return SegSelfAttnFn.apply(qkv2d, n_heads, segs, p_drop)


_XFUSED_FWD = os.environ.get("VALOR_ATTN_XFUSED_FWD", "0") == "1"


class SegCrossAttnFn(Function):

    @staticmethod
    def forward(ctx, q2d, kv, n_heads, segs, p_drop, dkv_buf=None):
        ctx.dkv_buf = dkv_buf
        R, E = q2d.shape
        q2d = q2d.contiguous()
        o = torch.empty((R, E), dtype=q2d.dtype, device=q2d.device)
        lses, rng = [], []
        for (r0, B, T, kv_range, kv_bmod) in segs:
            seed = off = 0
            if p_drop > 0:
                seed, off = DropoutState.draw_elems(B * n_heads * T * kv.shape[1])
            lses.append(torch.empty((B, n_heads, T), dtype=torch.float32, device=q2d.device)); rng.append((seed, off))
        fused = False
        if _XFUSED_FWD and len(segs) <= 2 and len({sg[4] for sg in segs}) == 1:
            fs = [dict(q=q2d[r0:r0 + B * T].view(B, T, E), o=o[r0:r0 + B * T].view(B, T, E), lse=lse, kv_range=kv_range, seed=seed, offset=off)
                  for (r0, B, T, kv_range, kv_bmod), lse, (seed, off) in zip(segs, lses, rng)]
            fused = K.cross_attn_fwd_fused(fs, kv[:, :, :E], kv[:, :, E:], n_heads, segs[0][4] or segs[0][1], scale=1.0 / math.sqrt(64),
                                           p_drop=p_drop)
        for (r0, B, T, kv_range, kv_bmod), lse, (seed, off) in zip(segs, lses, rng):
            if fused:
                break
            K.attn_fwd(q2d[r0:r0 + B * T].view(B, T, E), kv[:, :, :E], kv[:, :, E:], n_heads, kv_range=kv_range, kv_bmod=kv_bmod,
                       scale=1.0 / math.sqrt(64), p_drop=p_drop, seed=seed, offset=off, o=o[r0:r0 + B * T].view(B, T, E), lse=lse)
        ctx.save_for_backward(q2d, kv, o, *lses)
        ctx.cfg = (n_heads, segs, p_drop, rng)
        ctx.static_gen = StaticGen.seen(kv)
        return o

    @staticmethod
    def backward(ctx, do):
        StaticGen.check(ctx.static_gen)
        q2d, kv, o, *lses = ctx.saved_tensors
        n_heads, segs, p_drop, rng = ctx.cfg
        E = q2d.shape[1]
        do = do.contiguous()
        dq = torch.empty_like(q2d)
        dkv = ctx.dkv_buf if ctx.dkv_buf is not None else torch.empty_like(kv)
        if len(segs) <= 2 and len({sg[4] for sg in segs}) == 1:
            fs = [dict(q=q2d[r0:r0 + B * T].view(B, T, E), o=o[r0:r0 + B * T].view(B, T, E), dout=do[r0:r0 + B * T].view(B, T, E),
                       dq=dq[r0:r0 + B * T].view(B, T, E), lse=lse, kv_range=kv_range, seed=seed, offset=off)
                  for (r0, B, T, kv_range, kv_bmod), lse, (seed, off) in zip(segs, lses, rng)]
            if K.cross_attn_bwd_fused(fs, kv[:, :, :E], kv[:, :, E:], dkv[:, :, :E], dkv[:, :, E:], n_heads, segs[0][4] or segs[0][1],
                                      scale=1.0 / math.sqrt(64), p_drop=p_drop):
                return dq, dkv, None, None, None, None
        for i, ((r0, B, T, kv_range, kv_bmod), lse, (seed, off)) in enumerate(zip(segs, lses, rng)):
            sl = slice(r0, r0 + B * T)
            K.attn_bwd(q2d[sl].view(B, T, E), kv[:, :, :E], kv[:, :, E:], o[sl].view(B, T, E), lse, do[sl].view(B, T, E), n_heads,
                       dq=dq[sl].view(B, T, E), dk=dkv[:, :, :E], dv=dkv[:, :, E:], kv_range=kv_range, kv_bmod=kv_bmod,
                       scale=1.0 / math.sqrt(64), p_drop=p_drop, seed=seed, offset=off, accumulate_kv=i > 0)
        return dq, dkv, None, None, None, None


def seg_cross_attention(q2d, kv, n_heads, segs, p_drop=0.0, dkv_buf=None):
    return SegCrossAttnFn.apply(q2d, kv, n_heads, segs, p_drop, dkv_buf)


_ROWS_HWM = {}


def _rows_with_slack(n, cols, dtype, device):
    key = (cols, dtype, str(device))
    rows = max(_ROWS_HWM.get(key, 0), (n + n // 8 + 511) // 512 * 512)
    _ROWS_HWM[key] = rows
    return torch.empty((rows, cols), dtype=dtype, device=device)[:n]


class DecoderXentFn(Function):

    @staticmethod
    def forward(ctx, h, w_emb, dec_bias, labels, seg_rows, w_rows, smoothing, want_logits):
        n, V = h.shape[0], w_emb.shape[0]
        Vpad = (V + 31) // 32 * 32
        buf = _rows_with_slack(n, Vpad, h.dtype, h.device)
        logits = buf[:, :V]
        K.gemm(h, w_emb, bias=dec_bias, out=logits)
        loss_rows = torch.empty(n, dtype=torch.float32, device=h.device)
        lse = torch.empty(n, dtype=torch.float32, device=h.device)
        ctx.smoothing = float(smoothing)
        if w_rows is None:
            lib.call("valor_xent_smooth_fwd", _st(), _dt(h), _p(buf), _p(labels), _p(loss_rows), _p(lse), n, V, Vpad, ctx.smoothing)
        else:
            lib.call("valor_xent_fwd", _st(), _dt(h), _p(buf), _p(labels), _p(loss_rows), _p(lse), n, V, Vpad)
        losses, r0 = [], 0
        for nr in seg_rows:
            l = torch.empty((), dtype=torch.float32, device=h.device)
            if w_rows is None:
                lib.call("valor_mean_f32", _st(), _p(loss_rows[r0:r0 + nr]), nr, _p(l))
            else:
                lib.call("valor_weighted_mean_f32", _st(), _p(loss_rows[r0:r0 + nr]), _p(w_rows[r0:r0 + nr]), nr, _p(l))
            losses.append(l); r0 += nr
        ctx.save_for_backward(h, w_emb, labels, lse, buf, w_rows)
        ctx.V, ctx.seg_rows = V, tuple(seg_rows)
        ctx.params = (w_emb, dec_bias)
        extra = ((loss_rows,) if w_rows is not None else ()) + ((logits,) if want_logits else ())
        ctx.mark_non_differentiable(*extra)
        return (*losses, *extra)

    @staticmethod
    def backward(ctx, *douts):
        h, w_emb, labels, lse, buf, w_rows = ctx.saved_tensors
        V, Vpad = ctx.V, buf.shape[1]
        r0 = 0
        for nr, dl in zip(ctx.seg_rows, douts):
            g = dl.to(torch.float32).contiguous() if dl is not None else torch.zeros((), dtype=torch.float32, device=h.device)
            rows = slice(r0, r0 + nr)
            if w_rows is None:
                lib.call("valor_xent_smooth_bwd", _st(), _dt(h), _p(buf[rows]), _p(labels[rows]), _p(lse[rows]), _p(g), 1.0 / nr,
                         nr, V, Vpad, ctx.smoothing)
            else:
                lib.call("valor_xent_weighted_bwd", _st(), _dt(h), _p(buf[rows]), _p(labels[rows]), _p(lse[rows]), _p(w_rows[rows]), _p(g),
                         1.0 / nr, nr, V, Vpad)
            r0 += nr
        dlog = buf[:, :V]
        dh = K.gemm(dlog, w_emb, trans_b=True)
        dw, db = _wgrad_bgrad(dlog, h, *ctx.params, ctx.needs_input_grad[1], ctx.needs_input_grad[2], fuse=False)
        return dh, dw, db, None, None, None, None, None


def decoder_xent_segments(h, w_emb, dec_bias, labels, seg_rows, smoothing=0.0):
    return DecoderXentFn.apply(h, w_emb, dec_bias, labels, seg_rows, None, smoothing, False)


def decoder_xent_weighted_segments(h, w_emb, dec_bias, labels, seg_rows, w_rows, loss_rows_out=None):
    *losses, rows = DecoderXentFn.apply(h, w_emb, dec_bias, labels, seg_rows, w_rows, 0.0, False)
    if loss_rows_out is not None:
        loss_rows_out.append(rows)
    return tuple(losses)


def decoder_xent(h, w_emb, dec_bias, labels, want_logits=False, smoothing=0.0):
    out = DecoderXentFn.apply(h, w_emb, dec_bias, labels, [h.shape[0]], None, smoothing, want_logits)
    return out if want_logits else out[0]


def decoder_logits(h, w_emb, dec_bias):
    return K.gemm(h, w_emb, bias=dec_bias)


_FINE_CHUNK = int(os.environ.get("VALOR_FINE_CHUNK", "128"))


class FineContrastFn(Function):

    @staticmethod
    def forward(ctx, featA, featB, wA_raw, wB_raw, maskA, maskB, k):
        B, T, D = featA.shape
        Nv = featB.shape[1]
        dev = featA.device
        f32 = dict(dtype=torch.float32, device=dev)
        fa, fb = featA.contiguous().view(B * T, D), featB.contiguous().view(B * Nv, D)
        fused = featA.dtype == torch.bfloat16 and D % 64 == 0 and lib.load().valor_fine_set_fused(-1) == 1
        ldS = (B * Nv + 7) // 8 * 8
        wA, wB = torch.empty((B, T), **f32), torch.empty((B, Nv), **f32)
        lib.call("valor_fine_weight_softmax", _st(), _p(wA_raw), _p(maskA), _p(wA), B, T)
        lib.call("valor_fine_weight_softmax", _st(), _p(wB_raw), _p(maskB), _p(wB), B, Nv)
        score = torch.empty((B, B), **f32)
        A2B, B2A = torch.empty((B, B, T), **f32), torch.empty((B, B, Nv), **f32)
        idxA = torch.empty((B, B, T), dtype=torch.uint8, device=dev)
        idxB = torch.empty((B, B, Nv), dtype=torch.uint8, device=dev)
        if fused:
            lib.call("valor_fine_fused_fwd", _st(), _p(fa), _p(fb), _p(maskA), _p(maskB), _p(wA), _p(wB), _p(score), _p(A2B), _p(B2A),
                     _p(idxA), _p(idxB), B, B, T, Nv, D)
        else:
            S = torch.empty((B * T, ldS), **f32)
            K.gemm(fa, fb, out=S[:, :B * Nv], out_dtype=torch.float32)
            lib.call("valor_fine_reduce_fwd", _st(), _p(S), ldS, _p(maskA), _p(maskB), _p(wA), _p(wB), _p(score), _p(A2B),
                     _p(B2A), _p(idxA), _p(idxB), B, T, Nv)
        lse_r, lse_c = torch.empty(B, **f32), torch.empty(B, **f32)
        loss = torch.empty((), **f32)
        kk = k.detach().to(torch.float32).contiguous()
        lib.call("valor_infonce_fwd", _st(), _p(score), _p(kk), _p(lse_r), _p(lse_c), _p(loss), B)
        ctx.save_for_backward(fa, fb, maskA, maskB, wA, wB, score, A2B, B2A, idxA, idxB, lse_r, lse_c, kk)
        ctx.dims = (B, T, Nv, D, ldS, featA.dtype, fused)
        ctx.score = score
        return loss

    @staticmethod
    def backward(ctx, dloss):
        fa, fb, maskA, maskB, wA, wB, score, A2B, B2A, idxA, idxB, lse_r, lse_c, kk = ctx.saved_tensors
        B, T, Nv, D, ldS, fdt, fused = ctx.dims
        dev = fa.device
        f32 = dict(dtype=torch.float32, device=dev)
        g = dloss.to(torch.float32).contiguous()
        dscore, dk = torch.empty((B, B), **f32), torch.empty((), **f32)
        part = torch.empty(256, **f32)
        lib.call("valor_infonce_bwd", _st(), _p(score), _p(kk), _p(lse_r), _p(lse_c), _p(g), _p(dscore), _p(dk), _p(part), B)
        dwA, dwB = torch.empty((B, T), **f32), torch.empty((B, Nv), **f32)
        if fused:
            lib.call("valor_fine_weight_grad", _st(), _p(dscore), _p(A2B), _p(B2A), _p(dwA), _p(dwB), B, T, Nv)
            ch = min(B, max(1, _FINE_CHUNK))
            nch = (B + ch - 1) // ch
            dS = torch.empty((ch * T, ldS), dtype=fdt, device=dev)
            if ldS != B * Nv:
                dS[:, B * Nv:].zero_()
            dfa = torch.empty((B * T, D), dtype=fdt, device=dev)
            dfb = None
# ... 477 lines not shown
```

Baseline: 578.4.

## Add fused two-segment cross-attn forward kernel that stores dropout keep bitmasks for backward

Adds a 512-thread fused cross-attention forward kernel that handles both query segments in one launch and double-buffers K/V tiles through LDS. When dropout is active it packs per-element keep decisions into bitmasks via wave ballots and writes them to global memory, so the backward kernel reads those bits instead of regenerating the Philox dropout hash. The fused forward and keep-bit paths are now on by default, and the fallback threshold is lowered to Skv>=64. In exchange it adds extra global memory for the keep bitmasks and their writes and reads, plus more code paths.

```diff
diff --git a/include/valor_hip.h b/include/valor_hip.h
--- a/include/valor_hip.h
+++ b/include/valor_hip.h
@@ -68,6 +68,13 @@
 int valor_cross_attn_bwd_fused(void* stream, int dtype, const valor_xattn_seg* segs, int nseg, const void* k, const void* v, void* dk, void* dv,
                                int H, int Skv, int kv_bmod, int64_t k_bs, int64_t k_rs, int64_t v_bs, int64_t v_rs, int64_t dk_bs,
                                int64_t dk_rs, int64_t dv_bs, int64_t dv_rs, float scale, float p_drop, const uint64_t* rng_base);
+int valor_cross_attn_fwd_fused_keep(void* stream, int dtype, const valor_xattn_seg* segs, int nseg, const void* k, const void* v, int H, int Skv,
+                                    int kv_bmod, int64_t k_bs, int64_t k_rs, int64_t v_bs, int64_t v_rs, float scale, float p_drop,
+                                    const uint64_t* rng_base, void* keep0, void* keep1);
+int valor_cross_attn_bwd_fused_keep(void* stream, int dtype, const valor_xattn_seg* segs, int nseg, const void* k, const void* v, void* dk,
+                                    void* dv, int H, int Skv, int kv_bmod, int64_t k_bs, int64_t k_rs, int64_t v_bs, int64_t v_rs, int64_t dk_bs,
+                                    int64_t dk_rs, int64_t dv_bs, int64_t dv_rs, float scale, float p_drop, const uint64_t* rng_base,
+                                    const void* keep0, const void* keep1);
 
 int valor_ln_part_blocks(void);
 int valor_ln_set_variant(int v);
diff --git a/valor_amd/csrc/attention_x.hip b/valor_amd/csrc/attention_x.hip
--- a/valor_amd/csrc/attention_x.hip
+++ b/valor_amd/csrc/attention_x.hip
@@ -223,6 +223,246 @@
         }
         __syncthreads();
     }
+}
+
+template <int L> DEVINL uint32_t x_writelane(uint32_t old, uint32_t val) {
+    asm("v_writelane_b32 %0, %1, %2" : "+v"(old) : "s"(val), "n"(L));
+    return old;
+}
+template <int NH, bool DROP, bool KEEPW>
+__global__ __launch_bounds__(512, 2) void attn_x_fwd2_kernel(XuArgs p) {
+    const uint64_t rng_off0 = rng_offset(p.s[0].offset, p.rng_base), rng_off1 = rng_offset(p.s[1].offset, p.rng_base);
+    extern __shared__ __attribute__((aligned(16))) char smem[];
+    const int tid = threadIdx.x, lane = tid & 63;
+    const int wv = __builtin_amdgcn_readfirstlane(tid >> 6);
+    const int wave = wv & 3, grp = wv >> 2;
+    const int fr = lane & 15, g = lane >> 4;
+    const int h = blockIdx.x, kvb = blockIdx.y;
+
+    const rsrc_t rsK = x_head_rsrc(p.k, (int64_t)kvb * p.k_bs + h * ATT_D, p.Skv, p.k_rs);
+    const rsrc_t rsV = x_head_rsrc(p.v, (int64_t)kvb * p.v_bs + h * ATT_D, p.Skv, p.v_rs);
+    const int krs_b = (int)p.k_rs * 2, vrs_b = (int)p.v_rs * 2;
+
+    auto stage = [&](char* sK, char* sV, int kv0) {
+        const int prow = lane >> 3, pch = (lane & 7) ^ prow;
+#pragma unroll
+        for (int i = 0; i < 2; ++i) {
+            const int j = wv * 2 + i;
+            glds16(rsK, sK + j * 1024, (kv0 + j * 8 + prow) * krs_b + pch * 16);
+            glds16(rsV, sV + j * 1024, (kv0 + j * 8 + prow) * vrs_b + pch * 16);
+        }
+    };
+    stage(smem + 16384, smem, 0);
+
+    int sq0_[NH], ss0_[NH], ss1_[NH];
+    bool sv_[NH];
+    uint32_t hk_[NH], kpo_[NH];
+    bf16x8_t qf[NH][2];
+    f32x4_t oacc[NH][4];
+    float mrow[NH], lrow[NH];
+#pragma unroll
+    for (int u = 0; u < NH; ++u) {
+        const XuSub t_ = xu_sub(p, 2 * u + grp, kvb);
+        const XuSeg& sg = t_.seg ? p.s[1] : p.s[0];
+        sq0_[u] = t_.q0; ss0_[u] = t_.start; ss1_[u] = t_.end; sv_[u] = t_.valid;
+        hk_[u] = DROP ? attn_drop_headkey(sg.seed, t_.seg ? rng_off1 : rng_off0, t_.b * p.H + h) : 0u;
+        kpo_[u] = KEEPW ? xu_keep_base(p, t_.seg, t_.b, h, t_.q0) : 0u;
+        const int qr = t_.q0 + fr;
+#pragma unroll
+        for (int dg = 0; dg < 2; ++dg) {
+            u32x4_t z = {0u, 0u, 0u, 0u};
+            if (t_.valid && qr < sg.Sq)
+                z = *(const u32x4_t*)((const bf16_t*)sg.q + (int64_t)t_.b * sg.q_bs + (int64_t)qr * sg.q_rs + h * ATT_D + dg * 32 + g * 8);
+            qf[u][dg] = __builtin_bit_cast(bf16x8_t, z);
+        }
+        mrow[u] = -1e30f; lrow[u] = 0.f;
+#pragma unroll
+        for (int dt = 0; dt < 4; ++dt) oacc[u][dt] = (f32x4_t){0.f, 0.f, 0.f, 0.f};
+    }
+    const float sl2 = p.scale * LOG2E_F;
+    const uint32_t thr = drop_threshold(p.p_drop);
+    const float keep_scale = p.p_drop > 0.f ? 1.0f / (1.0f - p.p_drop) : 1.0f;
+    int troff[4];
+#pragma unroll
+    for (int dt = 0; dt < 4; ++dt) troff[dt] = tr_lane_off(lane, dt);
+    const int kw0 = wave * 32;
+    const int NT = (p.Skv + 127) >> 7;
+    const int sqpad0 = (p.s[0].Sq + 15) & ~15, sqpad1 = (p.s[1].Sq + 15) & ~15;
+
+    auto tile = [&](const int t, auto stage_c) {
+        constexpr int STG = decltype(stage_c)::value;
+        const int kv0 = t << 7;
+        char* sV = smem + STG * 32768;
+        char* sK = sV + 16384;
+        asm volatile("s_waitcnt vmcnt(0)" ::: "memory");
+        __syncthreads();
+        if (t + 1 < NT) {
+            char* nV = smem + (STG ^ 1) * 32768;
+            stage(nV + 16384, nV, kv0 + 128);
+        }
+        const int ka = kv0 + kw0;
+        if (ka < p.Skv) {
+            bf16x8_t kf[2][2], vfr[4];
+#pragma unroll
+            for (int kt = 0; kt < 2; ++kt)
+#pragma unroll
+                for (int dg = 0; dg < 2; ++dg) kf[kt][dg] = read_frag<bf16_t>(sK, kw0 + kt * 16 + fr, dg * 4 + g);
+            {
+                TrPair tv[4];
+#pragma unroll
+                for (int dt = 0; dt < 4; ++dt) x_tr_issue(tv[dt], sV + kw0 * TILE_ROW_BYTES + troff[dt]);
+                x_tr_wait4(tv);
+#pragma unroll
+                for (int dt = 0; dt < 4; ++dt) vfr[dt] = tr_frag(tv[dt]);
+            }
+#pragma unroll
+            for (int u = 0; u < NH; ++u) {
+                const int rs0 = ss0_[u], rs1 = ss1_[u];
+                if (!sv_[u] || ka + 32 <= rs0 || ka >= rs1) continue;
+                f32x4_t sacc[2];
+#pragma unroll
+                for (int kt = 0; kt < 2; ++kt) {
+                    sacc[kt] = (f32x4_t){0.f, 0.f, 0.f, 0.f};
+#pragma unroll
+                    for (int dg = 0; dg < 2; ++dg) sacc[kt] = Mma<bf16_t>::mma(kf[kt][dg], qf[u][dg], sacc[kt]);
+                }
+                float mx = -INFINITY;
+                if (ka >= rs0 && ka + 32 <= rs1) {
+#pragma unroll
+                    for (int kt = 0; kt < 2; ++kt) {
+                        sacc[kt] *= sl2;
+                        mx = fmaxf(mx, fmaxf(fmaxf(sacc[kt][0], sacc[kt][1]), fmaxf(sacc[kt][2], sacc[kt][3])));
+                    }
+                } else {
+#pragma unroll
+                    for (int kt = 0; kt < 2; ++kt)
+#pragma unroll
+                        for (int r = 0; r < 4; ++r) {
+                            const int key = ka + kt * 16 + 4 * g + r;
+                            const float s = (key >= rs0 && key < rs1) ? sacc[kt][r] * sl2 : -INFINITY;
+                            sacc[kt][r] = s;
+                            mx = fmaxf(mx, s);
+                        }
+                }
+                mx = fmaxf(mx, __shfl_xor(mx, 16, 64));
+                mx = fmaxf(mx, __shfl_xor(mx, 32, 64));
+                const float mnew = fmaxf(mrow[u], mx);
+                const float alpha = x_exp2(mrow[u] - mnew);
+                mrow[u] = mnew;
+                float ps = 0.f;
+                const int qr = sq0_[u] + fr;
+                const uint32_t hk = hk_[u];
+                const uint32_t rowbase = (uint32_t)qr * (uint32_t)p.Skv;
+                uint64_t km[KEEPW ? 8 : 1];
+#pragma unroll
+                for (int kt = 0; kt < 2; ++kt) {
+                    const f32x4_t sm = sacc[kt] - mnew;
+#pragma unroll
+                    for (int r = 0; r < 4; ++r) {
+                        float pv = x_exp2(sm[r]);
+                        ps += pv;
+                        if (DROP) {
+                            const int kloc = ka + kt * 16 + 4 * g + r - rs0;
+                            const bool keep = attn_drop_bits(hk, rowbase + (uint32_t)kloc) >= thr;
+                            pv = keep ? pv * keep_scale : 0.f;
+                            if (KEEPW) km[KEEPW ? kt * 4 + r : 0] = __builtin_amdgcn_ballot_w64(keep);
+                        }
+                        sacc[kt][r] = pv;
+                    }
+                }
+                if (DROP && KEEPW) {
+                    uint32_t kb = 0u;
+#define X_WL(E_) kb = x_writelane<2 * E_>(kb, (uint32_t)km[E_]); kb = x_writelane<2 * E_ + 1>(kb, (uint32_t)(km[E_] >> 32))
+                    X_WL(0); X_WL(1); X_WL(2); X_WL(3); X_WL(4); X_WL(5); X_WL(6); X_WL(7);
+#undef X_WL
+                    uint32_t* kp = (2 * u + grp >= p.n0) ? p.s[1].keep : p.s[0].keep;
+                    const int sqpad = (2 * u + grp >= p.n0) ? sqpad1 : sqpad0;
+                    if (lane < 16) kp[kpo_[u] + (uint32_t)((ka >> 5) * sqpad + lane)] = kb;
+                }
+                lrow[u] = lrow[u] * alpha + ps;
+                const bf16x8_t pf = pack_bf16x8(sacc[0], sacc[1]);
+#pragma unroll
+                for (int dt = 0; dt < 4; ++dt) {
+                    oacc[u][dt] *= alpha;
+                    oacc[u][dt] = Mma<bf16_t>::mma(vfr[dt], pf, oacc[u][dt]);
+                }
+            }
+        }
+    };
+    for (int t = 0; t < NT; t += 2) {
+        tile(t, std::integral_constant<int, 0>{});
+        if (t + 1 < NT) tile(t + 1, std::integral_constant<int, 1>{});
+    }
+    __syncthreads();
+
+    float* sO = (float*)(smem + grp * 32768);
+    float* sM = (float*)(smem + 65536 + grp * 1024);
+#pragma unroll
+    for (int u0 = 0; u0 < NH; u0 += 2) {
+#pragma unroll
+        for (int sl = 0; sl < 2; ++sl) {
+            if (u0 + sl >= NH) continue;
+            const int u = u0 + sl;
+            if (sv_[u]) {
+                float l = lrow[u];
+                l += __shfl_xor(l, 16, 64);
+                l += __shfl_xor(l, 32, 64);
+                if (g == 0) { sM[sl * 128 + wave * 16 + fr] = mrow[u]; sM[sl * 128 + 64 + wave * 16 + fr] = l; }
+#pragma unroll
+                for (int dt = 0; dt < 4; ++dt)
+                    *(f32x4_t*)(sO + sl * 4096 + wave * 1024 + fr * 64 + (((dt * 4 + g) ^ fr) << 2)) = oacc[u][dt];
+            }
+        }
+        __syncthreads();
+#pragma unroll
+        for (int sl = 0; sl < 2; ++sl) {
+            if (u0 + sl >= NH) continue;
+            const int u = u0 + sl;
+            if (!sv_[u]) continue;
+            const XuSub t_ = xu_sub(p, 2 * u + grp, kvb);
+            const XuSeg& sg = t_.seg ? p.s[1] : p.s[0];
+            const float* sMs = sM + sl * 128;
+            float mw[4], M = -1e30f;
+#pragma unroll
+            for (int w = 0; w < 4; ++w) { mw[w] = sMs[w * 16 + fr]; M = fmaxf(M, mw[w]); }
+            float L = 0.f, f[4];
+#pragma unroll
+            for (int w = 0; w < 4; ++w) { f[w] = x_exp2(mw[w] - M); L += sMs[64 + w * 16 + fr] * f[w]; }
+            const float inv = L > 0.f ? 1.0f / L : 0.f;
+            const int qr = t_.q0 + fr;
+            if (qr < sg.Sq) {
+                f32x4_t a = {0.f, 0.f, 0.f, 0.f};
+#pragma unroll
+                for (int w = 0; w < 4; ++w) a += *(const f32x4_t*)(sO + sl * 4096 + w * 1024 + fr * 64 + (((wave * 4 + g) ^ fr) << 2)) * f[w];
+                store4<bf16_t>((bf16_t*)sg.o + (int64_t)t_.b * sg.o_bs + (int64_t)qr * sg.o_rs + h * ATT_D + wave * 16 + 4 * g, a * inv);
+                if (wave == 0 && g == 0) ((float*)sg.lse)[((int64_t)t_.b * p.H + h) * sg.Sq + qr] = (M + __log2f(L)) * LN2_F;
+            }
+        }
+        if (u0 + 2 < NH) __syncthreads();
+    }
+}
+
+void attn_x_fwd2_launch(hipStream_t st, const XuArgs& p) {
+    dim3 grid(p.H, p.bmod);
+    const size_t lds = 65536 + 2048;
+    const bool keepw = p.p_drop > 0.f && p.s[0].keep != nullptr;
+#define X_FWD2_I(N_, D_, K_)                                                                                        \
+    do {                                                                                                            \
+        static bool attr_set = false;                                                                               \
+        if (!attr_set) {                                                                                            \
+            hipFuncSetAttribute((const void*)attn_x_fwd2_kernel<N_, D_, K_>, hipFuncAttributeMaxDynamicSharedMemorySize, (int)lds); \
+            attr_set = true;                                                                                        \
+        }                                                                                                           \
+        hipLaunchKernelGGL((attn_x_fwd2_kernel<N_, D_, K_>), grid, dim3(512), lds, st, p);                          \
+    } while (0)
+#define X_FWD2(N_)                                                                                                  \
+    do {                                                                                                            \
+        if (p.p_drop > 0.f) { if (keepw) X_FWD2_I(N_, true, true); else X_FWD2_I(N_, true, false); }                \
+        else X_FWD2_I(N_, false, false);                                                                            \
+    } while (0)
+    if (p.nsub <= 6) X_FWD2(3); else X_FWD2(5);
+#undef X_FWD2
+#undef X_FWD2_I
 }
 
 template <int NQS, bool DROP, bool ACC>
@@ -493,7 +733,7 @@
 
 bool attn_x_fwd_launch(hipStream_t st, const AttnArgs& p) {
     const int n = x_nqs(p);
-    if (n <= 0 || n > 8 || p.Skv < 128) return false;
+    if (n <= 0 || n > 8 || p.Skv < 64) return false;
     const int bmod = p.kv_bmod > 0 ? p.kv_bmod : p.B;
     dim3 grid(p.H, bmod);
     static const int db = [] { const char* e = getenv("VALOR_XATTN_FWD_DB"); return e ? atoi(e) : 1; }();
diff --git a/valor_amd/csrc/attention_xu.hip b/valor_amd/csrc/attention_xu.hip
--- a/valor_amd/csrc/attention_xu.hip
+++ b/valor_amd/csrc/attention_xu.hip
@@ -1,42 +1,6 @@
 #include "attn_common.h"
 
-struct XuSeg {
-    const void* q; const void* o; const void* dout; void* dq; const float* lse; const int* kv_range;
-    int64_t q_bs, q_rs, o_bs, o_rs, do_bs, do_rs, dq_bs, dq_rs;
-    int B, Sq;
-    uint64_t seed, offset;
-};
-struct XuArgs {
-    XuSeg s[2];
-    const void* k; const void* v; void* dk; void* dv;
-    int64_t k_bs, k_rs, v_bs, v_rs, dk_bs, dk_rs, dv_bs, dv_rs;
-    int nseg, bmod, H, Skv;
-    int n0, qs0, qs1, nsub;
-    float scale, p_drop;
-    const uint64_t* rng_base;
-};
-
 DEVINL float xu_exp2(float x) { return __builtin_amdgcn_exp2f(x); }
-DEVINL rsrc_t xu_head_rsrc(const void* base, int64_t elem_off, int rows, int64_t rs) {
-    return make_rsrc((const bf16_t*)base + elem_off, (uint32_t)(((int64_t)(rows - 1) * rs + ATT_D) * 2));
-}
-
-struct XuSub { int seg, b, q0, start, end; bool valid; };
-DEVINL XuSub xu_sub(const XuArgs& p, int u, int kvb) {
-    XuSub s;
-    s.valid = u < p.nsub;
-    const int uu = s.valid ? u : 0;
-    s.seg = uu >= p.n0 ? 1 : 0;
-    const int ul = s.seg ? uu - p.n0 : uu;
-    const int qs = s.seg ? p.qs1 : p.qs0;
-    const int j = ul / qs;
-    s.b = kvb + j * p.bmod;
-    s.q0 = (ul - j * qs) * 16;
-    const int* kr = s.seg ? p.s[1].kv_range : p.s[0].kv_range;
-    s.start = 0; s.end = p.Skv;
-    if (kr) { s.start = kr[2 * s.b]; s.end = s.start + kr[2 * s.b + 1]; }
-    return s;
-}
 
 #ifdef ATT_STAMP
 #ifndef XU_STAMP_TILE
@@ -51,7 +15,7 @@
 #define XU_STAMP_AT(i)
 #endif
 
-template <int NQS, bool DROP>
+template <int NQS, bool DROP, bool KEEP>
 __global__ __launch_bounds__(256, 2) void attn_xu_bwd_kernel(XuArgs p) {
 #ifdef ATT_STAMP
     uint64_t stamp_[12] = {0, 0, 0, 0, 0, 0, 0, 0, 0, 0, 0, 0};
@@ -79,11 +43,14 @@
 
     int sb_[NQS], sq0_[NQS], ss0_[NQS], ss1_[NQS], sg_[NQS];
     bool sv_[NQS];
+    uint32_t kpo_[KEEP ? NQS : 1];
 #pragma unroll
     for (int u = 0; u < NQS; ++u) {
         const XuSub t_ = xu_sub(p, u, kvb);
         sb_[u] = t_.b; sq0_[u] = t_.q0; ss0_[u] = t_.start; ss1_[u] = t_.end; sv_[u] = t_.valid; sg_[u] = t_.seg;
-    }
+        if (KEEP) kpo_[KEEP ? u : 0] = xu_keep_base(p, t_.seg, t_.b, h, t_.q0);
+    }
+    const int sqpad0 = (p.s[0].Sq + 15) & ~15, sqpad1 = (p.s[1].Sq + 15) & ~15;
 
     {
         const int prow = lane >> 3, pch = (lane & 7) ^ prow;
@@ -144,6 +111,10 @@
     const int ds_r = (4 * g + (fr >> 2)) * 32 + 8 * (fr & 3);
     const int NT = (p.Skv + 63) >> 6;
     const int prow = lane >> 3, pch = (lane & 7) ^ prow;
+    const int kdw = ((wave & 1) * 4 + (fr & 3)) * 2 + (fr >> 3);
+    uint32_t kmask[4];
+#pragma unroll
+    for (int r = 0; r < 4; ++r) kmask[r] = 1u << (4 * g + 16 * ((fr >> 2) & 1) + r);
 
 #ifdef ATT_STAMP
     asm volatile("s_waitcnt vmcnt(0) lgkmcnt(0)" ::: "memory");
@@ -157,13 +128,24 @@
             const int j = wave * 2 + i;
             glds16(rsK, sK + j * 1024, (kv0 + j * 8 + prow) * krs_b + pch * 16);
             glds16(rsV, sV + j * 1024, (kv0 + j * 8 + prow) * vrs_b + pch * 16);
+        }
+        const int ka = kv0 + kw0;
+        uint32_t kbw[KEEP ? NQS : 1];
+        if (KEEP) {
+#pragma unroll
+            for (int u = 0; u < NQS; ++u) {
+                kbw[KEEP ? u : 0] = 0u;
+                if (sv_[u] && ka + 16 > ss0_[u] && ka < ss1_[u]) {
+                    const uint32_t* kp = sg_[u] ? p.s[1].keep : p.s[0].keep;
+                    kbw[KEEP ? u : 0] = kp[kpo_[KEEP ? u : 0] + (uint32_t)((ka >> 5) * (sg_[u] ? sqpad1 : sqpad0) + kdw)];
+                }
+            }
         }
         XU_STAMP_AT(1);
         asm volatile("s_waitcnt vmcnt(0)" ::: "memory");
         XU_STAMP_AT(2);
         __syncthreads();
         XU_STAMP_AT(3);
-        const int ka = kv0 + kw0;
         bf16x8_t kf[2], vf[2];
 #pragma unroll
         for (int dg = 0; dg < 2; ++dg) {
@@ -199,7 +181,7 @@
                     const int key = ka + fr;
                     const float kout = (key >= ss0_[u] && key < ss1_[u]) ? 0.f : INFINITY;
                     uint32_t hk = 0;
-                    if (DROP) {
+                    if (DROP && !KEEP) {
                         const XuSeg& sg = sg_[u] ? p.s[1] : p.s[0];
                         hk = attn_drop_headkey(sg.seed, (sg_[u] ? rng_off1 : rng_off0), sb_[u] * p.H + h);
                     }
@@ -211,7 +193,8 @@
                         float dp = pacc[r];
                         float pd = prb;
                         if (DROP) {
-                            const bool keep = attn_drop_bits(hk, (row0 + r) * (uint32_t)p.Skv + (uint32_t)(key - ss0_[u])) >= thr;
+                            const bool keep = KEEP ? (kbw[KEEP ? u : 0] & kmask[r]) != 0u
+                                                   : attn_drop_bits(hk, (row0 + r) * (uint32_t)p.Skv + (uint32_t)(key - ss0_[u])) >= thr;
                             dp = keep ? dp * keep_scale : 0.f;
                             pd = keep ? prb * keep_scale : 0.f;
                         }
@@ -289,171 +272,6 @@
 #endif
 }
 
-DEVINL int xu_p_off(int fr, int b) { return fr * 128 + ((((b >> 4) ^ fr) & 7) << 4) + ((b & 8) ^ ((fr & 8))); }
-
-template <int NQS, bool DROP>
-__global__ __launch_bounds__(256, 2) void attn_xu_fwd_kernel(XuArgs p) {
-    const uint64_t rng_off0 = rng_offset(p.s[0].offset, p.rng_base), rng_off1 = rng_offset(p.s[1].offset, p.rng_base);
-    extern __shared__ __attribute__((aligned(16))) char smem[];
-    constexpr int QIMG = NQS * 16 * TILE_ROW_BYTES;
-    char* sQ = smem;
-    char* sKV = smem + QIMG;
-    char* sP = sKV + 32768;
-    float* sMax = (float*)(sP + NQS * 2048);
-    float* sSum = sMax + NQS * 64;
-    const int tid = threadIdx.x, lane = tid & 63;
-    const int wave = __builtin_amdgcn_readfirstlane(tid >> 6);
-    const int fr = lane & 15, g = lane >> 4;
-    const int h = blockIdx.x, kvb = blockIdx.y;
-
-    const rsrc_t rsK = xu_head_rsrc(p.k, (int64_t)kvb * p.k_bs + h * ATT_D, p.Skv, p.k_rs);
-    const rsrc_t rsV = xu_head_rsrc(p.v, (int64_t)kvb * p.v_bs + h * ATT_D, p.Skv, p.v_rs);
-    const int krs_b = (int)p.k_rs * 2, vrs_b = (int)p.v_rs * 2;
-    const int prow = lane >> 3, pch = (lane & 7) ^ prow;
-
-    int sb_[NQS], sq0_[NQS], ss0_[NQS], ss1_[NQS], sg_[NQS];
-    bool sv_[NQS];
-#pragma unroll
-    for (int u = 0; u < NQS; ++u) {
-        const XuSub t_ = xu_sub(p, u, kvb);
-        sb_[u] = t_.b; sq0_[u] = t_.q0; ss0_[u] = t_.start; ss1_[u] = t_.end; sv_[u] = t_.valid; sg_[u] = t_.seg;
-    }
-    for (int pc = wave; pc < 2 * NQS; pc += 4) {
-        const int u = pc >> 1, piece = pc & 1;
-        const XuSub su = xu_sub(p, u, kvb);
-        const XuSeg& sg = su.seg ? p.s[1] : p.s[0];
-        if (su.valid) {
-            const rsrc_t rq = xu_head_rsrc(sg.q, (int64_t)su.b * sg.q_bs + h * ATT_D, sg.Sq, sg.q_rs);
-            glds16(rq, sQ + pc * 1024, (su.q0 + piece * 8 + prow) * (int)(sg.q_rs * 2) + pch * 16);
-        } else {
-            *(u32x4_t*)(sQ + pc * 1024 + lane * 16) = (u32x4_t){0u, 0u, 0u, 0u};
-        }
-    }
-    auto stage = [&](int t, char* buf) {
-        const int kv0 = t << 6;
-#pragma unroll
-        for (int i = 0; i < 2; ++i) {
-            const int j = wave * 2 + i;
-            glds16(rsK, buf + j * 1024, (kv0 + j * 8 + prow) * krs_b + pch * 16);
-            glds16(rsV, buf + 8192 + j * 1024, (kv0 + j * 8 + prow) * vrs_b + pch * 16);
-        }
-    };
-    const int NT = (p.Skv + 63) >> 6;
-    stage(0, sKV);
-
-    f32x4_t oacc[NQS];
-    float mrow[NQS], lrow[NQS];
-#pragma unroll
-    for (int u = 0; u < NQS; ++u) { oacc[u] = (f32x4_t){0.f, 0.f, 0.f, 0.f}; mrow[u] = -1e30f; lrow[u] = 0.f; }
-    const float sl2 = p.scale * LOG2E_F;
-    const uint32_t thr = drop_threshold(p.p_drop);
-    const float keep_scale = p.p_drop > 0.f ? 1.0f / (1.0f - p.p_drop) : 1.0f;
-    const int troff_w = tr_lane_off(lane, wave);
-    const int kw0 = wave * 16;
-    const int po[4] = {xu_p_off(fr, 8 * g), xu_p_off(fr, 8 * g + 32), xu_p_off(fr, 8 * g + 64), xu_p_off(fr, 8 * g + 96)};
-
-    for (int t = 0; t < NT; ++t) {
-        const int kv0 = t << 6;
-        char* const cur = sKV + (t & 1) * 16384;
-        asm volatile("s_waitcnt vmcnt(0)" ::: "memory");
-        __syncthreads();
-        if (t + 1 < NT) stage(t + 1, sKV + ((t + 1) & 1) * 16384);
-        const int ka = kv0 + kw0;
-        bf16x8_t kf[2];
-#pragma unroll
-        for (int dg = 0; dg < 2; ++dg) kf[dg] = read_frag<bf16_t>(cur, kw0 + fr, dg * 4 + g);
-        f32x4_t sv4[NQS];
-#pragma unroll
-        for (int u = 0; u < NQS; ++u) {
-            const bool actt = sv_[u] && kv0 + 64 > ss0_[u] && kv0 < ss1_[u];
-            if (!actt) continue;
-            float mx = -INFINITY;
-            sv4[u] = (f32x4_t){-INFINITY, -INFINITY, -INFINITY, -INFINITY};
-            if (ka + 16 > ss0_[u] && ka < ss1_[u]) {
-                f32x4_t sacc = {0.f, 0.f, 0.f, 0.f};
-#pragma unroll
-                for (int dg = 0; dg < 2; ++dg) sacc = Mma<bf16_t>::mma(kf[dg], read_frag<bf16_t>(sQ, u * 16 + fr, dg * 4 + g), sacc);
-#pragma unroll
-                for (int r = 0; r < 4; ++r) {
-                    const int key = ka + 4 * g + r;
-                    const float s = (key >= ss0_[u] && key < ss1_[u]) ? sacc[r] * sl2 : -INFINITY;
-                    sv4[u][r] = s;
-                    mx = fmaxf(mx, s);
-                }
-                mx = fmaxf(mx, __shfl_xor(mx, 16, 64));
-                mx = fmaxf(mx, __shfl_xor(mx, 32, 64));
-            }
-            if (g == 0) sMax[u * 64 + wave * 16 + fr] = mx;
-        }
-        __syncthreads();
-        float alpha[NQS];
-#pragma unroll
-        for (int u = 0; u < NQS; ++u) {
-            alpha[u] = 1.0f;
-            const bool actt = sv_[u] && kv0 + 64 > ss0_[u] && kv0 < ss1_[u];
-            if (!actt) continue;
-            const float* mp = sMax + u * 64 + fr;
-            const float mt = fmaxf(fmaxf(mp[0], mp[16]), fmaxf(mp[32], mp[48]));
-            const float mnew = fmaxf(mrow[u], mt);
-            alpha[u] = xu_exp2(mrow[u] - mnew);
-            mrow[u] = mnew;
-            float ps = 0.f;
-            f32x4_t pv;
-            uint32_t hk = 0;
-            if (DROP) {
-                const XuSeg& sg = sg_[u] ? p.s[1] : p.s[0];
-                hk = attn_drop_headkey(sg.seed, (sg_[u] ? rng_off1 : rng_off0), sb_[u] * p.H + h);
-            }
-            const uint32_t rowbase = (uint32_t)(sq0_[u] + fr) * (uint32_t)p.Skv;
-#pragma unroll
-            for (int r = 0; r < 4; ++r) {
-                float e = xu_exp2(sv4[u][r] - mnew);
-                ps += e;
-                if (DROP) e = attn_drop_bits(hk, rowbase + (uint32_t)(ka + 4 * g + r - ss0_[u])) >= thr ? e * keep_scale : 0.f;
-                pv[r] = e;
-            }
-            ps += __shfl_xor(ps, 16, 64);
-            ps += __shfl_xor(ps, 32, 64);
-            lrow[u] = lrow[u] * alpha[u] + ps;
-            *(u32x2_t*)(sP + u * 2048 + xu_p_off(fr, (kw0 + 4 * g) * 2)) = (u32x2_t){pack2_bf16(pv[0], pv[1]), pack2_bf16(pv[2], pv[3])};
-        }
-        __syncthreads();
-        {
-            const bf16x8_t vt0 = read_frag_tr_nat(cur + 8192, 0, troff_w), vt1 = read_frag_tr_nat(cur + 8192, 32, troff_w);
-#pragma unroll
-            for (int u = 0; u < NQS; ++u) {
-                if (!(sv_[u] && kv0 + 64 > ss0_[u] && kv0 < ss1_[u])) continue;
-                const char* b = sP + u * 2048;
-                const u32x2_t a0 = *(const u32x2_t*)(b + po[0]), a1 = *(const u32x2_t*)(b + po[1]), a2 = *(const u32x2_t*)(b + po[2]),
-                              a3 = *(const u32x2_t*)(b + po[3]);
-                const bf16x8_t p0 = __builtin_bit_cast(bf16x8_t, (u32x4_t){a0[0], a0[1], a1[0], a1[1]});
-                const bf16x8_t p1 = __builtin_bit_cast(bf16x8_t, (u32x4_t){a2[0], a2[1], a3[0], a3[1]});
-                oacc[u] *= alpha[u];
-                oacc[u] = Mma<bf16_t>::mma(vt0, p0, oacc[u]);
-                oacc[u] = Mma<bf16_t>::mma(vt1, p1, oacc[u]);
-            }
-        }
-    }
-    __syncthreads();
-#pragma unroll
-    for (int u = 0; u < NQS; ++u)
-        if (g == 0) sSum[u * 64 + wave * 16 + fr] = lrow[u];
-    __syncthreads();
-#pragma unroll
-    for (int u = 0; u < NQS; ++u) {
-        if (!sv_[u]) continue;
-        const XuSeg& sg = sg_[u] ? p.s[1] : p.s[0];
-        const float* lp = sSum + u * 64 + fr;
-        const float L = (lp[0] + lp[16]) + (lp[32] + lp[48]);
-        const float inv = L > 0.f ? 1.0f / L : 0.f;
-        const int qr = sq0_[u] + fr;
-        if (qr < sg.Sq) {
-            store4<bf16_t>((bf16_t*)sg.o + (int64_t)sb_[u] * sg.o_bs + (int64_t)qr * sg.o_rs + h * ATT_D + 16 * wave + 4 * g, oacc[u] * inv);
-            if (wave == 0 && g == 0) ((float*)sg.lse)[((int64_t)sb_[u] * p.H + h) * sg.Sq + qr] = (mrow[u] + __log2f(L)) * LN2_F;
-        }
-    }
-}
-
 static int g_xu_on = [] { const char* e = getenv("VALOR_ATTN_XFUSED"); return e ? atoi(e) : 1; }();
 
 struct valor_xattn_seg_c {
@@ -464,7 +282,7 @@
 };
 
 static int xu_fill(XuArgs& p, int dtype, const void* segs_, int nseg, const void* k, const void* v, int H, int Skv, int kv_bmod, int64_t k_bs,
-                   int64_t k_rs, int64_t v_bs, int64_t v_rs, float scale, float p_drop, bool bwd) {
+                   int64_t k_rs, int64_t v_bs, int64_t v_rs, float scale, float p_drop, bool bwd, void* const* keep) {
     const valor_xattn_seg_c* segs = (const valor_xattn_seg_c*)segs_;
     if (dtype != VALOR_DT_BF16 || !g_xu_on) return VALOR_ERR_ARG;
     if (!segs || nseg < 1 || nseg > 2 || !k || !v || H <= 0 || Skv < 64 || kv_bmod <= 0) return VALOR_ERR_ARG;
@@ -488,6 +306,9 @@
         d.q = s.q; d.o = s.o; d.dout = s.dout; d.dq = s.dq; d.lse = s.lse; d.kv_range = s.kv_range;
         d.q_bs = s.q_bs; d.q_rs = s.q_rs; d.o_bs = s.o_bs; d.o_rs = s.o_rs; d.do_bs = s.do_bs; d.do_rs = s.do_rs; d.dq_bs = s.dq_bs; d.dq_rs = s.dq_rs;
         d.B = s.B; d.Sq = s.Sq; d.seed = s.seed; d.offset = s.offset;
+        d.keep = (uint32_t*)(keep ? keep[i] : nullptr);
+        if (keep && (keep[0] != nullptr) != (keep[i] != nullptr)) return VALOR_ERR_ARG;
+        if (d.keep && (((uintptr_t)d.keep & 15) || (int64_t)s.B * H * (2 * ((Skv + 63) >> 6)) * ((s.Sq + 15) & ~15) >= lim)) return VALOR_ERR_ARG;
         const int qs = (s.Sq + 15) >> 4, n = (s.B / kv_bmod) * qs;
         if (i == 0) { p.qs0 = qs; p.n0 = n; } else p.qs1 = qs;
         nsub += n;
@@ -498,58 +319,67 @@
     return VALOR_OK;
 }
 
+static int xu_fwd(void* stream, int dtype, const void* segs, int nseg, const void* k, const void* v, int H, int Skv, int kv_bmod, int64_t k_bs,
+                  int64_t k_rs, int64_t v_bs, int64_t v_rs, float scale, float p_drop, const uint64_t* rng_base, void* keep0, void* keep1) {
+    XuArgs p = {};
+    void* const keep[2] = {keep0, nseg > 1 ? keep1 : keep0};
+    const int rc = xu_fill(p, dtype, segs, nseg, k, v, H, Skv, kv_bmod, k_bs, k_rs, v_bs, v_rs, scale, p_drop, false, keep);
+    if (rc != VALOR_OK) return rc;
+    p.rng_base = rng_base;
+    attn_x_fwd2_launch((hipStream_t)stream, p);
+    return valor_launch_status();
+}
 extern "C" int valor_cross_attn_fwd_fused(void* stream, int dtype, const void* segs, int nseg, const void* k, const void* v, int H, int Skv,
                                           int kv_bmod, int64_t k_bs, int64_t k_rs, int64_t v_bs, int64_t v_rs, float scale, float p_drop,
                                           const uint64_t* rng_base) {
-    XuArgs p = {};
-    const int rc = xu_fill(p, dtype, segs, nseg, k, v, H, Skv, kv_bmod, k_bs, k_rs, v_bs, v_rs, scale, p_drop, false);
-    if (rc != VALOR_OK) return rc;
-    p.rng_base = rng_base;
-    hipStream_t st = (hipStream_t)stream;
-    dim3 grid(H, kv_bmod);
-    const int nsub = p.nsub;
-#define XUF_I(N_, D_)                                                                                               \
-    do {                                                                                                            \
-        const size_t lds = 2 * N_ * 2048 + 32768 + 2 * N_ * 256;                                                    \
-        static bool attr_set = false;                                                                               \
-        if (!attr_set) {                                                                                            \
-            hipFuncSetAttribute((const void*)attn_xu_fwd_kernel<N_, D_>, hipFuncAttributeMaxDynamicSharedMemorySize, (int)lds); \
-            attr_set = true;                                                                                        \
-        }                                                                                                           \
-        hipLaunchKernelGGL((attn_xu_fwd_kernel<N_, D_>), grid, dim3(256), lds, st, p);                              \
-    } while (0)
-#define XUF(N_) do { if (p_drop > 0.f) XUF_I(N_, true); else XUF_I(N_, false); } while (0)
-    if (nsub <= 4) XUF(4); else if (nsub <= 6) XUF(6); else if (nsub <= 8) XUF(8); else XUF(10);
-#undef XUF
-#undef XUF_I
-    return valor_launch_status();
-}
-
-extern "C" int valor_cross_attn_bwd_fused(void* stream, int dtype, const void* segs, int nseg, const void* k, const void* v, void* dk, void* dv,
-                                          int H, int Skv, int kv_bmod, int64_t k_bs, int64_t k_rs, int64_t v_bs, int64_t v_rs, int64_t dk_bs,
-                                          int64_t dk_rs, int64_t dv_bs, int64_t dv_rs, float scale, float p_drop, const uint64_t* rng_base) {
+    return xu_fwd(stream, dtype, segs, nseg, k, v, H, Skv, kv_bmod, k_bs, k_rs, v_bs, v_rs, scale, p_drop, rng_base, nullptr, nullptr);
+}
+extern "C" int valor_cross_attn_fwd_fused_keep(void* stream, int dtype, const void* segs, int nseg, const void* k, const void* v, int H, int Skv,
+                                               int kv_bmod, int64_t k_bs, int64_t k_rs, int64_t v_bs, int64_t v_rs, float scale, float p_drop,
+                                               const uint64_t* rng_base, void* keep0, void* keep1) {
+    return xu_fwd(stream, dtype, segs, nseg, k, v, H, Skv, kv_bmod, k_bs, k_rs, v_bs, v_rs, scale, p_drop, rng_base, keep0, keep1);
+}
+
+static int xu_bwd(void* stream, int dtype, const void* segs, int nseg, const void* k, const void* v, void* dk, void* dv, int H, int Skv, int kv_bmod,
+                  int64_t k_bs, int64_t k_rs, int64_t v_bs, int64_t v_rs, int64_t dk_bs, int64_t dk_rs, int64_t dv_bs, int64_t dv_rs, float scale,
+                  float p_drop, const uint64_t* rng_base, const void* keep0, const void* keep1) {
     if (!dk || !dv || (dk_rs & 3) || (dv_rs & 3) || (dk_bs & 3) || (dv_bs & 3)) return VALOR_ERR_ARG;
     XuArgs p = {};
-    const int rc = xu_fill(p, dtype, segs, nseg, k, v, H, Skv, kv_bmod, k_bs, k_rs, v_bs, v_rs, scale, p_drop, true);
+    void* const keep[2] = {(void*)keep0, (void*)(nseg > 1 ? keep1 : keep0)};
+    const int rc = xu_fill(p, dtype, segs, nseg, k, v, H, Skv, kv_bmod, k_bs, k_rs, v_bs, v_rs, scale, p_drop, true, keep);
     if (rc != VALOR_OK) return rc;
     p.dk = dk; p.dv = dv; p.rng_base = rng_base;
     p.dk_bs = dk_bs; p.dk_rs = dk_rs; p.dv_bs = dv_bs; p.dv_rs = dv_rs;
     const int nsub = p.nsub;
+    const bool keepr = p_drop > 0.f && keep0 != nullptr;
     hipStream_t st = (hipStream_t)stream;
     const int n_items = H * kv_bmod;
-#define XU_I(N_, D_)                                                                                                \
+#define XU_I(N_, D_, K_)                                                                                            \
     do {                                                                                                            \
         const size_t lds = 3 * N_ * 2048 + 16384 + N_ * 128;                                                        \
         static bool attr_set = false;                                                                               \
         if (!attr_set) {                                                                                            \
-            hipFuncSetAttribute((const void*)attn_xu_bwd_kernel<N_, D_>, hipFuncAttributeMaxDynamicSharedMemorySize, (int)lds); \
+            hipFuncSetAttribute((const void*)attn_xu_bwd_kernel<N_, D_, K_>, hipFuncAttributeMaxDynamicSharedMemorySize, (int)lds); \
             attr_set = true;                                                                                        \
         }                                                                                                           \
-        hipLaunchKernelGGL((attn_xu_bwd_kernel<N_, D_>), dim3(n_items), dim3(256), lds, st, p);                     \
+        hipLaunchKernelGGL((attn_xu_bwd_kernel<N_, D_, K_>), dim3(n_items), dim3(256), lds, st, p);                 \
     } while (0)
-#define XU(N_) do { if (p_drop > 0.f) XU_I(N_, true); else XU_I(N_, false); } while (0)
+#define XU(N_) do { if (p_drop > 0.f) { if (keepr) XU_I(N_, true, true); else XU_I(N_, true, false); } else XU_I(N_, false, false); } while (0)
     if (nsub <= 4) XU(4); else if (nsub <= 6) XU(6); else if (nsub <= 8) XU(8); else XU(10);
 #undef XU
 #undef XU_I
     return valor_launch_status();
 }
+extern "C" int valor_cross_attn_bwd_fused(void* stream, int dtype, const void* segs, int nseg, const void* k, const void* v, void* dk, void* dv,
+                                          int H, int Skv, int kv_bmod, int64_t k_bs, int64_t k_rs, int64_t v_bs, int64_t v_rs, int64_t dk_bs,
+                                          int64_t dk_rs, int64_t dv_bs, int64_t dv_rs, float scale, float p_drop, const uint64_t* rng_base) {
+    return xu_bwd(stream, dtype, segs, nseg, k, v, dk, dv, H, Skv, kv_bmod, k_bs, k_rs, v_bs, v_rs, dk_bs, dk_rs, dv_bs, dv_rs, scale, p_drop, rng_base,
+                  nullptr, nullptr);
+}
+extern "C" int valor_cross_attn_bwd_fused_keep(void* stream, int dtype, const void* segs, int nseg, const void* k, const void* v, void* dk, void* dv,
+                                               int H, int Skv, int kv_bmod, int64_t k_bs, int64_t k_rs, int64_t v_bs, int64_t v_rs, int64_t dk_bs,
+                                               int64_t dk_rs, int64_t dv_bs, int64_t dv_rs, float scale, float p_drop, const uint64_t* rng_base,
+                                               const void* keep0, const void* keep1) {
+    return xu_bwd(stream, dtype, segs, nseg, k, v, dk, dv, H, Skv, kv_bmod, k_bs, k_rs, v_bs, v_rs, dk_bs, dk_rs, dv_bs, dv_rs, scale, p_drop, rng_base,
+                  keep0, keep1);
+}
diff --git a/valor_amd/csrc/attn_common.h b/valor_amd/csrc/attn_common.h
--- a/valor_amd/csrc/attn_common.h
+++ b/valor_amd/csrc/attn_common.h
@@ -75,7 +75,50 @@
 }
 DEVINL f32x4_t splat4(float x) { return (f32x4_t){x, x, x, x}; }
 
+struct XuSeg {
+    const void* q; const void* o; const void* dout; void* dq; const float* lse; const int* kv_range;
+    int64_t q_bs, q_rs, o_bs, o_rs, do_bs, do_rs, dq_bs, dq_rs;
+    int B, Sq;
+    uint64_t seed, offset;
+    uint32_t* keep;
+};
+struct XuArgs {
+    XuSeg s[2];
+    const void* k; const void* v; void* dk; void* dv;
+    int64_t k_bs, k_rs, v_bs, v_rs, dk_bs, dk_rs, dv_bs, dv_rs;
+    int nseg, bmod, H, Skv;
+    int n0, qs0, qs1, nsub;
+    float scale, p_drop;
+    const uint64_t* rng_base;
+};
+
+DEVINL rsrc_t xu_head_rsrc(const void* base, int64_t elem_off, int rows, int64_t rs) {
+    return make_rsrc((const bf16_t*)base + elem_off, (uint32_t)(((int64_t)(rows - 1) * rs + ATT_D) * 2));
+}
+
+struct XuSub { int seg, b, q0, start, end; bool valid; };
+DEVINL XuSub xu_sub(const XuArgs& p, int u, int kvb) {
+    XuSub s;
+    s.valid = u < p.nsub;
+    const int uu = s.valid ? u : 0;
+    s.seg = uu >= p.n0 ? 1 : 0;
+    const int ul = s.seg ? uu - p.n0 : uu;
+    const int qs = s.seg ? p.qs1 : p.qs0;
+    const int j = ul / qs;
+    s.b = kvb + j * p.bmod;
+    s.q0 = (ul - j * qs) * 16;
+    const int* kr = s.seg ? p.s[1].kv_range : p.s[0].kv_range;
+    s.start = 0; s.end = p.Skv;
+    if (kr) { s.start = kr[2 * s.b]; s.end = s.start + kr[2 * s.b + 1]; }
+    return s;
+}
+DEVINL uint32_t xu_keep_base(const XuArgs& p, int seg, int b, int h, int q0) {
+    const int sqpad = ((seg ? p.s[1].Sq : p.s[0].Sq) + 15) & ~15;
+    return (uint32_t)((b * p.H + h) * (2 * ((p.Skv + 63) >> 6)) * sqpad + q0);
+}
+
 bool attn_res_fwd_launch(hipStream_t st, const AttnArgs& p);
 bool attn_res_bwd_launch(hipStream_t st, const AttnArgs& p);
 bool attn_x_fwd_launch(hipStream_t st, const AttnArgs& p);
 bool attn_x_bwd_launch(hipStream_t st, const AttnArgs& p);
+void attn_x_fwd2_launch(hipStream_t st, const XuArgs& p);
diff --git a/valor_amd/kernels.py b/valor_amd/kernels.py
--- a/valor_amd/kernels.py
+++ b/valor_amd/kernels.py
@@ -378,24 +378,43 @@
     return True
 
 
-def cross_attn_fwd_fused(segs, k, v, n_heads, kv_bmod, *, scale=0.125, p_drop=0.0):
+def xattn_keep_bits(B, n_heads, T, Skv, device):
+    return torch.empty((B, n_heads, 2 * ((Skv + 63) // 64), (T + 15) // 16 * 16), dtype=torch.int32, device=device)
+
+
+def _xattn_keep(segs, keep, n_heads, Skv):
+    assert len(keep) == len(segs)
+    for sg, kb in zip(segs, keep):
+        _check_gpu(kb)
+        B, T = sg["q"].shape[:2]
+        assert kb.dtype == torch.int32 and kb.is_contiguous() and kb.shape == (B, n_heads, 2 * ((Skv + 63) // 64), (T + 15) // 16 * 16)
+    return _ptr(keep[0]), _ptr(keep[-1])
+
+
+def cross_attn_fwd_fused(segs, k, v, n_heads, kv_bmod, *, scale=0.125, p_drop=0.0, keep=None):
     if not _xattn_domain(segs, k, kv_bmod):
         return False
     import ctypes
     arr = _xattn_segs(segs, kv_bmod, False)
     kb, kr = _bsr(k); vb, vr = _bsr(v)
-    return _xattn_call("valor_cross_attn_fwd_fused", _stream(), DT_BF16, ctypes.cast(arr, ctypes.c_void_p), len(segs), _ptr(k), _ptr(v),
-                       n_heads, k.shape[1], int(kv_bmod), kb, kr, vb, vr, float(scale), float(p_drop), RNG_BASE)
-
-
-def cross_attn_bwd_fused(segs, k, v, dk, dv, n_heads, kv_bmod, *, scale=0.125, p_drop=0.0):
+    args = (_stream(), DT_BF16, ctypes.cast(arr, ctypes.c_void_p), len(segs), _ptr(k), _ptr(v), n_heads, k.shape[1], int(kv_bmod), kb, kr, vb, vr,
+            float(scale), float(p_drop), RNG_BASE)
+    if keep is None:
+        return _xattn_call("valor_cross_attn_fwd_fused", *args)
+    return _xattn_call("valor_cross_attn_fwd_fused_keep", *args, *_xattn_keep(segs, keep, n_heads, k.shape[1]))
+
+
+def cross_attn_bwd_fused(segs, k, v, dk, dv, n_heads, kv_bmod, *, scale=0.125, p_drop=0.0, keep=None):
     if not _xattn_domain(segs, k, kv_bmod):
         return False
     arr = _xattn_segs(segs, kv_bmod, True)
     kb, kr = _bsr(k); vb, vr = _bsr(v); dkb, dkr = _bsr(dk); dvb, dvr = _bsr(dv)
     import ctypes
-    return _xattn_call("valor_cross_attn_bwd_fused", _stream(), DT_BF16, ctypes.cast(arr, ctypes.c_void_p), len(segs), _ptr(k), _ptr(v), _ptr(dk),
-                       _ptr(dv), n_heads, k.shape[1], int(kv_bmod), kb, kr, vb, vr, dkb, dkr, dvb, dvr, float(scale), float(p_drop), RNG_BASE)
+    args = (_stream(), DT_BF16, ctypes.cast(arr, ctypes.c_void_p), len(segs), _ptr(k), _ptr(v), _ptr(dk), _ptr(dv), n_heads, k.shape[1],
+            int(kv_bmod), kb, kr, vb, vr, dkb, dkr, dvb, dvr, float(scale), float(p_drop), RNG_BASE)
+    if keep is None:
+        return _xattn_call("valor_cross_attn_bwd_fused", *args)
+    return _xattn_call("valor_cross_attn_bwd_fused_keep", *args, *_xattn_keep(segs, keep, n_heads, k.shape[1]))
 
 
 def win_attn_fwd(qkv, geo, table, n_heads, B):
diff --git a/valor_amd/lib.py b/valor_amd/lib.py
--- a/valor_amd/lib.py
+++ b/valor_amd/lib.py
@@ -96,6 +96,9 @@
                        _vp, _i64, _i64, _vp, _i, _f, _f, _u64, _u64, _i, _vp],
     "valor_cross_attn_fwd_fused": [_vp, _i, _vp, _i, _vp, _vp, _i, _i, _i, _i64, _i64, _i64, _i64, _f, _f, _vp],
     "valor_cross_attn_bwd_fused": [_vp, _i, _vp, _i, _vp, _vp, _vp, _vp, _i, _i, _i, _i64, _i64, _i64, _i64, _i64, _i64, _i64, _i64, _f, _f, _vp],
+    "valor_cross_attn_fwd_fused_keep": [_vp, _i, _vp, _i, _vp, _vp, _i, _i, _i, _i64, _i64, _i64, _i64, _f, _f, _vp, _vp, _vp],
+    "valor_cross_attn_bwd_fused_keep": [_vp, _i, _vp, _i, _vp, _vp, _vp, _vp, _i, _i, _i, _i64, _i64, _i64, _i64, _i64, _i64, _i64, _i64, _f, _f, _vp,
+                                        _vp, _vp],
     "valor_reducer_unique_id": [_vp],
     "valor_reducer_create": [_vp, _vp, _i, _i, _i, _vp, _vp, _vp, _i, _i],
     "valor_reducer_launch_bucket": [_vp, _i, _vp, _i],
diff --git a/valor_amd/ops.py b/valor_amd/ops.py
--- a/valor_amd/ops.py
+++ b/valor_amd/ops.py
@@ -566,7 +566,12 @@
     return SegSelfAttnFn.apply(qkv2d, n_heads, segs, p_drop)
 
 
-_XFUSED_FWD = os.environ.get("VALOR_ATTN_XFUSED_FWD", "0") == "1"
+def _xfused_fwd():
+    return os.environ.get("VALOR_ATTN_XFUSED_FWD", "1") != "0"
+
+
+def _xkeep():
+    return os.environ.get("VALOR_ATTN_XKEEP", "1") != "0"
 
 
 class SegCrossAttnFn(Function):
@@ -583,18 +588,22 @@
             if p_drop > 0:
                 seed, off = DropoutState.draw_elems(B * n_heads * T * kv.shape[1])
             lses.append(torch.empty((B, n_heads, T), dtype=torch.float32, device=q2d.device)); rng.append((seed, off))
-        fused = False
-        if _XFUSED_FWD and len(segs) <= 2 and len({sg[4] for sg in segs}) == 1:
+        fused, keep = False, None
+        if _xfused_fwd() and len(segs) <= 2 and len({sg[4] for sg in segs}) == 1:
+            if p_drop > 0 and _xkeep():
+                keep = [K.xattn_keep_bits(B, n_heads, T, kv.shape[1], q2d.device) for (r0, B, T, kv_range, kv_bmod) in segs]
             fs = [dict(q=q2d[r0:r0 + B * T].view(B, T, E), o=o[r0:r0 + B * T].view(B, T, E), lse=lse, kv_range=kv_range, seed=seed, offset=off)
                   for (r0, B, T, kv_range, kv_bmod), lse, (seed, off) in zip(segs, lses, rng)]
             fused = K.cross_attn_fwd_fused(fs, kv[:, :, :E], kv[:, :, E:], n_heads, segs[0][4] or segs[0][1], scale=1.0 / math.sqrt(64),
-                                           p_drop=p_drop)
+                                           p_drop=p_drop, keep=keep)
+        if not fused:
+            keep = None
         for (r0, B, T, kv_range, kv_bmod), lse, (seed, off) in zip(segs, lses, rng):
             if fused:
                 break
             K.attn_fwd(q2d[r0:r0 + B * T].view(B, T, E), kv[:, :, :E], kv[:, :, E:], n_heads, kv_range=kv_range, kv_bmod=kv_bmod,
                        scale=1.0 / math.sqrt(64), p_drop=p_drop, seed=seed, offset=off, o=o[r0:r0 + B * T].view(B, T, E), lse=lse)
-        ctx.save_for_backward(q2d, kv, o, *lses)
+        ctx.save_for_backward(q2d, kv, o, *lses, *(keep or []))
         ctx.cfg = (n_heads, segs, p_drop, rng)
         ctx.static_gen = StaticGen.seen(kv)
         return o
@@ -602,8 +611,9 @@
     @staticmethod
     def backward(ctx, do):
         StaticGen.check(ctx.static_gen)
-        q2d, kv, o, *lses = ctx.saved_tensors
+        q2d, kv, o, *rest = ctx.saved_tensors
         n_heads, segs, p_drop, rng = ctx.cfg
+        lses, keep = rest[:len(segs)], (rest[len(segs):] or None)
         E = q2d.shape[1]
         do = do.contiguous()
         dq = torch.empty_like(q2d)
@@ -613,7 +623,7 @@
                        dq=dq[r0:r0 + B * T].view(B, T, E), lse=lse, kv_range=kv_range, seed=seed, offset=off)
                   for (r0, B, T, kv_range, kv_bmod), lse, (seed, off) in zip(segs, lses, rng)]
             if K.cross_attn_bwd_fused(fs, kv[:, :, :E], kv[:, :, E:], dkv[:, :, :E], dkv[:, :, E:], n_heads, segs[0][4] or segs[0][1],
-                                      scale=1.0 / math.sqrt(64), p_drop=p_drop):
+                                      scale=1.0 / math.sqrt(64), p_drop=p_drop, keep=keep):
                 return dq, dkv, None, None, None, None
         for i, ((r0, B, T, kv_range, kv_bmod), lse, (seed, off)) in enumerate(zip(segs, lses, rng)):
             sl = slice(r0, r0 + B * T)
```

Measured after the change: 579.9, median of 6. About the same (+0.3%).
